# labicon/dp-ilqr

Measured on AMD Instinct MI355X. Metric: ilqr_subproblems_per_sec, higher is better.
Workload: dtype f64; 1 GPU; cfg2: batches of 1024 independent 5-agent DoubleIntDynamics4D iLQR sub-problems per GPU per step, T=50, scripts/analysis.py scenario distribution, tol=1e-3, n_lqr_iter=50; 2468 steps = 2527232 distinct seeds per GPU, window of 6144 in flight; 1 repetition(s) of the job on disjoint seeds, the median is reported; batch_per_gpu=1024, window=6144, n_x=20, n_u=10, horizon=50, parallelism=single GPU

## Files before the change

### dpilqr_amd/_lib.py

```python
import ctypes as C
import os
from pathlib import Path

HERE = Path(__file__).resolve().parent


def route_env(name):
    return os.environ.get(name) if os.environ.get("DPILQR_DEBUG_ROUTES") == "1" else None


def route_flag(name):
    return route_env(name) is not None


LIB_PATH = Path(route_env("DPILQR_LIB")) if route_env("DPILQR_LIB") else HERE / "libdpilqr_hip.so"

i32, i64, f64, vp = C.c_int32, C.c_int64, C.c_double, C.c_void_p

OK, EINVAL, EUNSUPPORTED, EHIP, ENOGPU, EWORKSPACE = 0, -1, -2, -3, -4, -5
N_ALPHA = 10
ABI_VERSION = 4
STATUS_ACTIVE, STATUS_CONVERGED, STATUS_LINESEARCH_FAILED, STATUS_MAX_ITER, STATUS_SINGULAR, STATUS_KILLED, STATUS_FAULT = 0, 1, 2, 3, 4, 5, 6


class BatchDesc(C.Structure):
    _fields_ = [("B", i32), ("k", i32), ("n_s", i32), ("n_c", i32), ("T", i32), ("uniform_model", i32),
                ("dt", f64), ("w_ref", f64), ("w_prox", f64),
                ("model", vp), ("model_bstride", i64), ("n_dims", vp), ("n_dims_bstride", i64),
                ("xf", vp), ("xf_bstride", i64), ("Q", vp), ("Q_bstride", i64), ("R", vp), ("R_bstride", i64),
                ("Qf", vp), ("Qf_bstride", i64), ("radius", vp), ("radius_bstride", i64)]


class DpilqrError(RuntimeError):
    def __init__(self, code, msg):
        super().__init__(f"libdpilqr_hip error {code}: {msg}")
        self.code = code


_DP = C.POINTER(BatchDesc)
SIGNATURES = {
    "dpilqr_abi_version": (i32, []),
    "dpilqr_last_error": (C.c_char_p, []),
    "dpilqr_device_info": (i32, [i32, C.POINTER(i32), C.POINTER(i32), C.c_char_p, i32]),
    "dpilqr_model_dims": (i32, [i32, C.POINTER(i32), C.POINTER(i32)]),
    "dpilqr_model_f": (i32, [i32, i32, vp, vp, vp, vp, vp]),
    "dpilqr_model_integrate": (i32, [i32, i32, vp, vp, vp, f64, vp, vp]),
    "dpilqr_model_linearize": (i32, [i32, i32, vp, vp, vp, f64, vp, vp, vp]),
    "dpilqr_cost_eval": (i32, [_DP, i32, vp, vp, i32, vp, vp]),
    "dpilqr_tile_layout": (i32, [i32, i32, C.POINTER(i64 * 7), C.POINTER(i64 * 7), C.POINTER(i64)]),
    "dpilqr_make_tiles": (i32, [_DP, vp, vp, vp, vp, vp, vp]),
    "dpilqr_rollout": (i32, [_DP, vp, vp, vp, vp, vp]),
    "dpilqr_backward_pass_tiles": (i32, [i32, i32, i32, i32, vp, vp, vp, vp, vp, vp, vp, vp]),
    "dpilqr_backward_pass_tiles_blocks": (i32, [i32, i32, i32, i32, i32, i32, vp, vp, vp, vp, vp, vp, vp, vp]),
    "dpilqr_tiles_bytes": (i64, [i32, i32, i32, i32]),
    "dpilqr_backward_pass": (i32, [_DP, vp, vp, vp, vp, vp, vp, vp]),
    "dpilqr_backward_pass_fused": (i32, [_DP, vp, vp, vp, vp, vp, vp, vp]),
    "dpilqr_forward_pass": (i32, [_DP, vp, vp, vp, vp, vp, i32, vp, vp, vp, vp]),
    "dpilqr_alphas": (i32, [C.POINTER(f64 * N_ALPHA)]),
    "dpilqr_solve_workspace_bytes": (i64, [_DP, i32, i32]),
    "dpilqr_solver_create": (i32, [C.POINTER(vp)]),
    "dpilqr_solver_destroy": (i32, [vp]),
    "dpilqr_solver_set_progress": (i32, [vp, vp, vp]),
    "dpilqr_solve_batch": (i32, [vp, _DP, vp, vp, i32, f64, f64, i32, vp, i64, vp, vp, vp, vp, vp, vp, vp, vp, vp]),
    "dpilqr_solve_enqueue": (i32, [_DP, vp, vp, i32, f64, f64, i32, vp, i64, vp, vp, vp, vp, vp, vp, vp, vp, i32, i32, vp]),
    "dpilqr_solve_iterations_bound": (i64, [_DP, i32, i32]),
    "dpilqr_rollout_f32": (i32, [_DP, vp, vp, vp, vp, vp]),
    "dpilqr_backward_pass_workspace_bytes": (i64, [_DP, i32]),
    "dpilqr_backward_pass_f32": (i32, [_DP, vp, vp, vp, vp, vp, vp, vp]),
    "dpilqr_forward_pass_f32": (i32, [_DP, vp, vp, vp, vp, vp, i32, vp, vp, vp, vp]),
    "dpilqr_solve_workspace_bytes_f32": (i64, [_DP, i32, i32]),
    "dpilqr_solve_batch_f32": (i32, [vp, _DP, vp, vp, i32, f64, f64, i32, vp, i64, vp, vp, vp, vp, vp, vp, vp, vp, vp]),
    "dpilqr_debug_stamps": (i32, [vp]),
    "dpilqr_profile_enable": (i32, [vp, i32]),
    "dpilqr_profile_read": (i32, [vp, C.POINTER(f64 * 4), C.POINTER(i64 * 4), C.POINTER(i64 * 4), i32]),
    "dpilqr_profile_read_sweep": (i32, [vp, i32, C.POINTER(f64), C.POINTER(i64), C.POINTER(i64), i32]),
    "dpilqr_pairwise_graph": (i32, [i32, i32, i32, i32, vp, vp, vp, vp]),
    "dpilqr_dispatch_graph": (i32, [i32, i32, i32, i32, vp, vp, i64, vp, vp, vp, vp, vp, vp, vp, vp, vp]),
    "dpilqr_dispatch_gather": (i32, [i32, i32, i32, i32, i32, i32, vp, i32, i32, vp, vp, vp, vp, i64, vp, vp, vp, vp, vp]),
    "dpilqr_dispatch_gather_params": (i32, [i32, i32, i32, i32, vp, vp, vp, vp]),
    "dpilqr_dispatch_stitch": (i32, [i32, i32, i32, i32, i32, vp, vp, vp, vp, vp, vp, vp, vp]),
    "dpilqr_dispatch_pack_rows": (i32, [i32, i32, i32, i32, i32, vp, vp, vp, vp, vp, vp, vp, vp, i64, vp]),
    "dpilqr_dispatch_scatter_rows": (i32, [i64, i32, i32, i32, i32, vp, i64, vp, vp, vp]),
    "dpilqr_random_setup": (i32, [i32, i64, i32, i32, i32, f64, f64, vp, vp, vp]),
}

_PLAN = [_DP, vp, vp, vp]
_CLOSED_LOOP_ARGS = {"rollout": [i32] + [vp] * 9,
                     "advance": [i32, vp, i32, i32, i32] + [vp] * 12}
EXT_SIGNATURES = {f"dpilqr_policy_{kind}{form}": (i32, _PLAN + ([i32, vp] if "_dec" in form else []) + rest)
                  for kind, rest in _CLOSED_LOOP_ARGS.items() for form in ("", "_large", "_dec", "_dec_team")}
EXT_SIGNATURES["dpilqr_dispatch_stitch_policy"] = (i32, [i32, i32, i32, i32, i32, i32, vp, vp, vp, vp, vp, vp, vp, vp, vp, vp])

SWARM_SIGNATURES = {
    "dpilqr_dispatch_graph_wide": (i32, SIGNATURES["dpilqr_dispatch_graph"][1][:-1] + [i32, vp]),
    "dpilqr_dispatch_gather_wide": (i32, SIGNATURES["dpilqr_dispatch_gather"][1][:-1] + [i32, vp]),
    "dpilqr_dispatch_stitch_wide": (i32, SIGNATURES["dpilqr_dispatch_stitch"][1][:-1] + [i32, vp]),
    "dpilqr_rollout_wide": (i32, [_DP, vp, vp, vp, vp, vp, vp, vp]),
}

SWARM_POLICY_SIGNATURES = {
    "dpilqr_dispatch_stitch_policy_wide": (i32, EXT_SIGNATURES["dpilqr_dispatch_stitch_policy"][1][:-1] + [i32, vp]),
    "dpilqr_policy_rollout_dec_wide": (i32, EXT_SIGNATURES["dpilqr_policy_rollout_dec_team"][1][:-1] + [i32, vp]),
}

SWARM_ADVANCE_SIGNATURES = {
    "dpilqr_policy_advance_dec_wide": (i32, EXT_SIGNATURES["dpilqr_policy_advance_dec_team"][1][:-1] + [i32, vp]),
    "dpilqr_cost_eval_wide": (i32, list(SIGNATURES["dpilqr_cost_eval"][1])),
}

ORDER_SIGNATURES = {
    "dpilqr_cost_keys": (i32, [_DP, vp, vp, vp, vp, vp]),
    "dpilqr_order_list": (i32, [vp, vp, vp, i32, i32, i32, i32, vp, vp]),
    "dpilqr_order_position": (i32, [i32, i32, i32, i32, i32]),
}
ORDER_SPREAD, ORDER_GROUPED = 1, 2

_GW = SWARM_SIGNATURES["dpilqr_dispatch_graph_wide"][1]
NEAREST_SIGNATURES = {"dpilqr_dispatch_graph_nearest": (i32, _GW[:8] + [i32] + _GW[8:15] + [vp] + _GW[15:])}

SWARM_STUDY_SIGNATURES = {
    "dpilqr_trial_inputs": (i32, [i32, C.c_int64, vp, i32, i32, i32, C.c_double, C.c_double, i32, i32, i32, C.c_double, vp, vp, vp, vp, vp]),
}
TRIAL_INPUTS_LDS = 37888

SEPARATED_SIGNATURES = {
    "dpilqr_setup_separate": (i32, [i32, i32, i32, i32, C.c_double, C.c_double, i32, vp, vp, vp, vp]),
}
SETUP_SEPARATE_MAX_ITER = 4096
SETUP_SEPARATE_LDS = 8232

MAX_AGENTS = 64
MAX_TEAM = 256


class BucketResults(C.Structure):
    _fields_ = [("X", vp * (MAX_AGENTS + 1)), ("U", vp * (MAX_AGENTS + 1)), ("first", i32 * (MAX_AGENTS + 1)),
                ("count", i32 * (MAX_AGENTS + 1))]


class BucketGains(C.Structure):
    _fields_ = [("K", vp * (MAX_AGENTS + 1))]


_lib = None


def load():
    global _lib
    if _lib is None:
        if not LIB_PATH.exists():
            raise ImportError(f"{LIB_PATH} is missing: build it with `python -c 'import __graft_entry__ as g; g.build()'` "
                              "(hipcc --offload-arch=gfx950).  dpilqr_amd has no CPU fallback.")
        lib = C.CDLL(str(LIB_PATH))
        for name, (res, args) in {**SIGNATURES, **EXT_SIGNATURES, **SWARM_SIGNATURES, **SWARM_POLICY_SIGNATURES, **SWARM_ADVANCE_SIGNATURES,
                                   **ORDER_SIGNATURES, **NEAREST_SIGNATURES, **SWARM_STUDY_SIGNATURES, **SEPARATED_SIGNATURES}.items():
            fn = getattr(lib, name)
            fn.restype = res
            fn.argtypes = args
        if lib.dpilqr_abi_version() != ABI_VERSION:
            raise ImportError(f"{LIB_PATH}: ABI version {lib.dpilqr_abi_version()}, this binding is for {ABI_VERSION}")
        _lib = lib
    return _lib


def check(rc):
    if rc < 0:
        raise DpilqrError(rc, load().dpilqr_last_error().decode())
    return rc


def alphas():
    a = (f64 * N_ALPHA)()
    check(load().dpilqr_alphas(C.byref(a)))
    return list(a)


TILE_PARTS = ["A", "B", "Lxx", "Lux", "Luu", "Lx", "Lu"]


def tile_layout(n_x, n_u):
    off, ld = (i64 * 7)(), (i64 * 7)()
    stride = i64(0)
    check(load().dpilqr_tile_layout(n_x, n_u, C.byref(off), C.byref(ld), C.byref(stride)))
    return {p: (off[i], ld[i]) for i, p in enumerate(TILE_PARTS)}, stride.value


PROFILE_CLASSES = {"tiles": 1, "riccati": 2, "forward": 4, "rollout": 8}


def profile_enable(on=True, classes=None):
    mask = 0 if not classes else sum(PROFILE_CLASSES[c] for c in classes)
    return load().dpilqr_profile_enable(solver(), int(bool(on)) | (mask << 1))


def profile_read(reset=True):
    ms, ln, it = (f64 * 4)(), (i64 * 4)(), (i64 * 4)()
    check(load().dpilqr_profile_read(solver(), C.byref(ms), C.byref(ln), C.byref(it), int(bool(reset))))
    names = ["tiles", "riccati", "forward", "rollout"]
    return {n: dict(ms=ms[i], launches=ln[i], items=it[i]) for i, n in enumerate(names)}


def profile_read_sweep(waves, reset=True):
    ms, ln, it = f64(), i64(), i64()
    check(load().dpilqr_profile_read_sweep(solver(), int(waves), C.byref(ms), C.byref(ln), C.byref(it), int(bool(reset))))
    return dict(ms=ms.value, launches=ln.value, items=it.value)


import threading

_solvers = threading.local()


def solver():
    import torch
    dev = torch.cuda.current_device()
    table = getattr(_solvers, "table", None)
    if table is None:
        table = _solvers.table = {}
        import atexit
        atexit.register(_destroy_solvers, table)
    if dev not in table:
        h = vp()
        check(load().dpilqr_solver_create(C.byref(h)))
        table[dev] = h
    return table[dev]


PROGRESS_FN = C.CFUNCTYPE(None, vp, i32, i32)


class progress_callback:

    def __init__(self, fn):
        self.error = None

        def call(user, done, total):
            if self.error is not None:
                return
            try:
                fn(int(done), int(total))
            except BaseException as e:
                self.error = e

        self._c = PROGRESS_FN(call) if fn is not None else None

    def __enter__(self):
        if self._c is not None:
            check(load().dpilqr_solver_set_progress(solver(), C.cast(self._c, vp), None))
        return self

    def __exit__(self, *exc):
        if self._c is not None:
            check(load().dpilqr_solver_set_progress(solver(), None, None))
        if self.error is not None and exc[0] is None:
            raise self.error
        return False


def _destroy_solvers(table):
    lib = _lib
    if lib is not None:
        for h in table.values():
            lib.dpilqr_solver_destroy(h)
    table.clear()


_device_ok = None


def require_gpu():
    global _device_ok
    if _device_ok is None:
        import torch
        if not torch.cuda.is_available():
            raise DpilqrError(ENOGPU, "torch.cuda.is_available() is False: dpilqr_amd needs an MI355X (no CPU fallback)")
        check(load().dpilqr_device_info(torch.cuda.current_device(), None, None, None, 0))
        _device_ok = True
    return True
```

### dpilqr_amd/csrc/admit_order.hpp

```cpp
#pragma once
#include <cstdint>

#if defined(__HIPCC__)
#include <hip/hip_runtime.h>
#define DPILQR_HD __host__ __device__
#else
#define DPILQR_HD
#endif

namespace dpilqr {

enum CostOrder : int { kOrderOff = 0, kOrderSpread = 1, kOrderGrouped = 2 };
constexpr int kDefaultCostOrder = kOrderSpread;
enum CostKey : int { kKeyNearCount = 0, kKeyDenseSteps = 1 };
constexpr int kDefaultCostKey = kKeyDenseSteps;

constexpr int kOrderMinLive = 1024;
constexpr int kOrderClasses = 64;

struct SweepDeal {
    int n, n_cus, waves, per_layer, layers, rounds, lo, extra;
    DPILQR_HD SweepDeal(int n_, int n_cus_, int waves_) : n(n_), n_cus(n_cus_), waves(waves_) {
        const int lpr = waves / 4;
        per_layer = 4 * n_cus;
        layers = (n + per_layer - 1) / per_layer;
        rounds = (layers + lpr - 1) / lpr;
        lo = rounds > 0 ? layers / rounds : 0;
        extra = rounds > 0 ? layers - lo * rounds : 0;
    }
    DPILQR_HD int layers_of(int round) const { return lo + (round < extra ? 1 : 0); }
    DPILQR_HD int first_layer(int round) const { return round * lo + (round < extra ? round : extra); }
    DPILQR_HD int round_of_layer(int layer) const {
        const int head = extra * (lo + 1);
        return layer < head ? layer / (lo + 1) : extra + (layer - head) / (lo > 0 ? lo : 1);
    }
    DPILQR_HD int slot(int round, int cu, int wave) const {
        if (round >= rounds || wave >= 4 * layers_of(round)) return -1;
        const int s = (first_layer(round) + (wave >> 2)) * per_layer + (wave & 3) * n_cus + cu;
        return s < n ? s : -1;
    }
};

DPILQR_HD inline int order_position(int rank, const SweepDeal& D, int order) {
    if (order != kOrderGrouped) return rank;
    const int round = D.round_of_layer(rank / D.per_layer);
    const int f = D.first_layer(round), m = D.layers_of(round);
    const int q = rank - f * D.per_layer;
    int base = 4 * m, e = 0;
    if (round == D.rounds - 1) {
        const int rem = D.n - (D.layers - 1) * D.per_layer;
        base = 4 * (m - 1) + rem / D.n_cus;
        e = rem % D.n_cus;
    }
    int cu, w;
    if (q < e * (base + 1)) { cu = q / (base + 1); w = q - cu * (base + 1); }
    else { const int q2 = q - e * (base + 1), per = base > 0 ? base : 1; cu = e + q2 / per; w = q2 - (cu - e) * per; }
    return (f + (w >> 2)) * D.per_layer + (w & 3) * D.n_cus + cu;
}

DPILQR_HD inline int order_class(int key, int T) {
    const int top = T + 1;
    const int c = top < kOrderClasses ? key : (int)((int64_t)key * (kOrderClasses - 1) / top);
    return c < 0 ? 0 : (c > kOrderClasses - 1 ? kOrderClasses - 1 : c);
}

#if defined(__HIPCC__) && defined(DPILQR_ADMIT_ORDER_KERNELS)

constexpr int kKeyStagedAgents = 5;
__global__ void __launch_bounds__(256) k_cost_keys(const double* __restrict__ X, const double* __restrict__ radius, int64_t radius_bstride,
                                                   const int32_t* __restrict__ list, const int32_t* __restrict__ count, int B, int T, int k,
                                                   int min_live, int32_t* __restrict__ key, int32_t* __restrict__ key_dense) {
    __shared__ double2 sP[4][64 * kKeyStagedAgents];
    const int n = count ? *count : B;
    if (n <= min_live) return;
    const int wave = (int)threadIdx.x >> 6, lane = threadIdx.x & 63;
    const int pos = (int)blockIdx.x * 4 + wave;
    if (pos >= n) return;
    const int b = list ? list[pos] : pos;
    if (b < 0 || b >= B) return;
    const double r = radius[(int64_t)b * radius_bstride];
    const double lim = r * r * (1.0 + 1e-12);
    const int nx = 4 * k;
    const double* Xb = X + (int64_t)b * (T + 1) * nx;
    const bool staged = k <= kKeyStagedAgents;
    int cnt = 0, dense = 0;
    for (int t0 = 0; t0 <= T; t0 += 64) {
        const int rows = min(64, T + 1 - t0);
        bool near = false;
        if (staged) {
            const double2* src = reinterpret_cast<const double2*>(Xb + (int64_t)t0 * nx);
            for (int e = lane; e < rows * k; e += 64) sP[wave][e] = src[2 * e];
            __builtin_amdgcn_wave_barrier();
            asm volatile("" ::: "memory");
            if (lane < rows) {
                double2 p[kKeyStagedAgents];
#pragma unroll
                for (int i = 0; i < kKeyStagedAgents; ++i) p[i] = sP[wave][lane * k + min(i, k - 1)];
#pragma unroll
                for (int i = 0; i < kKeyStagedAgents; ++i)
#pragma unroll
                    for (int j = i + 1; j < kKeyStagedAgents; ++j) {
                        const double ddx = p[i].x - p[j].x, ddy = p[i].y - p[j].y;
                        const double s2 = ddx * ddx + ddy * ddy;
                        near = near || (j < k && !(s2 > lim));
                    }
            }
            __builtin_amdgcn_wave_barrier();
            asm volatile("" ::: "memory");
        } else if (lane < rows) {
            const double* row = Xb + (int64_t)(t0 + lane) * nx;
            for (int i = 0; i < k; ++i)
                for (int j = i + 1; j < k; ++j) {
                    const double ddx = row[4 * i] - row[4 * j], ddy = row[4 * i + 1] - row[4 * j + 1];
                    const double s2 = ddx * ddx + ddy * ddy;
                    near = near || !(s2 > lim);
                }
        }
        const unsigned long long mask = __builtin_amdgcn_ballot_w64(near);
        cnt += __popcll(mask);
        if (mask) dense = t0 + 64 - __clzll(mask);
    }
    if (lane == 0) {
        if (key) key[pos] = cnt;
        if (key_dense) key_dense[pos] = dense;
    }
}

__global__ void __launch_bounds__(1024) k_order_list(const int32_t* __restrict__ src, int32_t* __restrict__ dst, const int32_t* __restrict__ count,
                                                     const int32_t* __restrict__ key, int T, int n_cus, int waves, int order, int min_live) {
    static_assert(kOrderClasses == 64, "the prefix sums below are one wavefront's, a bin per lane");
    __shared__ int hist[kOrderClasses], cursor[kOrderClasses];
    const int n = *count;
    if (n <= min_live || order == kOrderOff) {
        for (int i = threadIdx.x; i < n; i += blockDim.x) dst[i] = src[i];
        return;
    }
    if (threadIdx.x < kOrderClasses) hist[threadIdx.x] = 0;
    __syncthreads();
    for (int i = threadIdx.x; i < n; i += blockDim.x) atomicAdd(&hist[kOrderClasses - 1 - order_class(key[i], T)], 1);
    __syncthreads();
    if (threadIdx.x < kOrderClasses) {
        const int own = hist[threadIdx.x];
        int run = own;
        for (int off = 1; off < kOrderClasses; off <<= 1) {
            const int below = __shfl_up(run, off);
            if ((int)threadIdx.x >= off) run += below;
        }
        cursor[threadIdx.x] = run - own;
    }
    __syncthreads();
    const SweepDeal deal(n, n_cus, waves);
    for (int i = threadIdx.x; i < n; i += blockDim.x) {
        const int rank = atomicAdd(&cursor[kOrderClasses - 1 - order_class(key[i], T)], 1);
        const int pos = order_position(rank, deal, order);
        if (pos >= 0 && pos < n) dst[pos] = src[i];
    }
}

#endif

}
```

### dpilqr_amd/csrc/dpilqr_hip.hip

```cpp
#include <hip/hip_runtime.h>

#include <cstdarg>
#include <cstdio>
#include <algorithm>
#include <cstdlib>
#include <cstring>
#include <new>
#include <vector>

#include "dpilqr_hip.h"
#include "admit_order.hpp"
#include "launch.hpp"
#include "models.hpp"
#include "tiles.hpp"

namespace dpilqr {

static thread_local char g_err[512] = "";

int32_t fail(int32_t code, const char* fmt, ...) {
    va_list ap;
    va_start(ap, fmt);
    vsnprintf(g_err, sizeof(g_err), fmt, ap);
    va_end(ap);
    return code;
}
const char* last_error() { return g_err; }

const char* route_env(const char* name) {
    static const bool open = [] { const char* g = std::getenv("DPILQR_DEBUG_ROUTES"); return g && g[0] == '1' && g[1] == 0; }();
    return open ? std::getenv(name) : nullptr;
}

int device_cus() {
    static int cus_of[64] = {0};
    int dev = 0;
    if (hipGetDevice(&dev) != hipSuccess || dev < 0 || dev >= 64) return 256;
    if (cus_of[dev] == 0) {
        int n = 0;
        if (hipDeviceGetAttribute(&n, hipDeviceAttributeMultiprocessorCount, dev) != hipSuccess || n <= 0) n = 256;
        cus_of[dev] = n;
    }
    return cus_of[dev];
}

}

using namespace dpilqr;

namespace {

constexpr int kMaxAgents = 64;

int family_nc(int ns) { return ns == 3 ? 2 : ns == 4 ? 2 : ns == 5 ? 2 : ns == 6 ? 3 : ns == 12 ? 4 : -1; }

int32_t check_family5(const dpilqr_batch_desc* d, bool f32) {
    if (d->n_s != 5) return DPILQR_OK;
    if (f32) return fail(DPILQR_EUNSUPPORTED, "the fp32 arm does not serve the five-state family (BikeDynamics5D)");
    if (d->k * d->n_s > 60)
        return fail(DPILQR_EUNSUPPORTED, "k=%d BikeDynamics5D agents (n_x=%d): the five-state family is served up to 12 agents (n_x <= 60)",
                    d->k, d->k * d->n_s);
    return DPILQR_OK;
}

int32_t check_desc(const dpilqr_batch_desc* d, int max_k = kMaxAgents) {
    if (!d) return fail(DPILQR_EINVAL, "desc is NULL");
    if (d->B < 0 || d->k < 1 || d->T < 1) return fail(DPILQR_EINVAL, "bad sizes B=%d k=%d T=%d", d->B, d->k, d->T);
    if (d->k > max_k) return fail(DPILQR_EUNSUPPORTED, "k=%d agents per sub-problem exceeds %d", d->k, max_k);
    if (family_nc(d->n_s) != d->n_c)
        return fail(DPILQR_EINVAL, "(n_s,n_c)=(%d,%d) is not a model family; expected (3,2),(4,2),(5,2),(6,3),(12,4)", d->n_s, d->n_c);
    if (d->B > 0 && (!d->model || !d->n_dims || !d->xf || !d->Q || !d->R || !d->Qf || !d->radius))
        return fail(DPILQR_EINVAL, "desc holds a NULL device pointer");
    const uintptr_t ints = reinterpret_cast<uintptr_t>(d->model) | reinterpret_cast<uintptr_t>(d->n_dims);
    const uintptr_t dbls = reinterpret_cast<uintptr_t>(d->xf) | reinterpret_cast<uintptr_t>(d->Q) | reinterpret_cast<uintptr_t>(d->R) |
                           reinterpret_cast<uintptr_t>(d->Qf) | reinterpret_cast<uintptr_t>(d->radius);
    if (d->B > 0 && (ints % alignof(int32_t) != 0 || dbls % alignof(double) != 0))
        return fail(DPILQR_EINVAL, "desc holds a device pointer that is not aligned to its element type");
    return check_family5(d, false);
}

hipStream_t as_stream(void* s) { return reinterpret_cast<hipStream_t>(s); }

void alpha_table(double* a) {
    static const uint32_t bits[DPILQR_N_ALPHA] = {0x3f800000u, 0x3f68ba2eu, 0x3f2ed9f7u, 0x3ed92350u, 0x3e5eda27u,
                                                  0x3dbd05a8u, 0x3d04808du, 0x3c19864au, 0x3b13029cu, 0x39e8ae70u};
    for (int i = 0; i < DPILQR_N_ALPHA; ++i) {
        float f;
        memcpy(&f, &bits[i], 4);
        a[i] = (double)f;
    }
}

__global__ void k_init_state(int B, double* mu, double* delta, int32_t* status, int32_t* n_bwd, int32_t* n_fwd,
                             int32_t* singular, int32_t* counts, int n_counts, double* alphas_dev, double a0, double a1,
                             double a2, double a3, double a4, double a5, double a6, double a7, double a8, double a9) {
    const int i = blockIdx.x * blockDim.x + threadIdx.x;
    if (i < B) {
        mu[i] = 1.0; delta[i] = 2.0; status[i] = DPILQR_STATUS_ACTIVE; n_bwd[i] = 0; n_fwd[i] = 0; singular[i] = 0;
    }
    if (i < n_counts) counts[i] = 0;
    if (i == 0) {
        alphas_dev[0] = a0; alphas_dev[1] = a1; alphas_dev[2] = a2; alphas_dev[3] = a3; alphas_dev[4] = a4;
        alphas_dev[5] = a5; alphas_dev[6] = a6; alphas_dev[7] = a7; alphas_dev[8] = a8; alphas_dev[9] = a9;
    }
}

__global__ void k_admit(int32_t* list, int32_t* count, int32_t* next_count, int32_t* admitted, int B, int window,
                        int32_t* mail, int want_prefix, int64_t* t_admit, const int32_t* fault) {
    const int base = *count, first = *admitted;
    const int n_new = min(B - first, window - base);
    __shared__ int lowest;
    if (threadIdx.x == 0) lowest = first;
    __syncthreads();
    for (int i = threadIdx.x; i < n_new; i += blockDim.x) list[base + i] = first + i;
    if (t_admit && n_new > 0) {
        const int64_t now = (int64_t)__builtin_amdgcn_s_memrealtime();
        for (int i = threadIdx.x; i < n_new; i += blockDim.x) t_admit[first + i] = now;
    }
    if (mail && want_prefix) {
        int lo = first;
        for (int i = threadIdx.x; i < base; i += blockDim.x) lo = min(lo, list[i]);
        for (int off = 32; off > 0; off >>= 1) lo = min(lo, __shfl_down(lo, off));
        if ((threadIdx.x & 63) == 0) atomicMin(&lowest, lo);
        __syncthreads();
    }
    if (threadIdx.x == 0) {
        *count = base + n_new; *admitted = first + n_new; *next_count = 0;
        if (mail) { mail[0] = base + n_new; mail[1] = first + n_new; mail[2] = want_prefix ? lowest : 0; mail[3] = *fault; }
    }
}

__global__ void k_copy_f64(int n, const double* src, double* dst) {
    const int i = blockIdx.x * blockDim.x + threadIdx.x;
    if (i < n) dst[i] = src[i];
}

__global__ void k_finish_status(int B, int32_t* status) {
    const int i = blockIdx.x * blockDim.x + threadIdx.x;
    if (i < B && status[i] == DPILQR_STATUS_ACTIVE) status[i] = DPILQR_STATUS_MAX_ITER;
}

constexpr int kCountRing = 4;

struct SolveShape {
    bool big;
    size_t elem;
    bool fused;
};

struct SolveWorkspace {
    size_t tiles, K, d, Xc, Uc, mu, delta, J_star, J_last, alphas, singular, lists, counts, t_admit, total;
    SolveWorkspace(const dpilqr_batch_desc& D, int W, bool gains_in_ws, SolveShape sh) {
        const size_t B = D.B, n = (size_t)D.k * D.n_s, m = (size_t)D.k * D.n_c, T = D.T, Wn = W, e = sh.elem;
        const TileLayout L((int)n, (int)m);
        auto al = [](size_t x) { return (x + 255) & ~(size_t)255; };
        size_t o = 0;
        tiles = o;    o = al(o + (sh.big ? e * Wn * (size_t)riccati_big_scratch_elems((int)n, (int)m)
                                         : (sh.fused ? 0 : sizeof(double) * Wn * (T + 1) * L.stride)));
        K = o;        o = al(o + (gains_in_ws ? e * Wn * T * m * n : 0));
        d = o;        o = al(o + (gains_in_ws ? e * Wn * T * m : 0));
        Xc = o;       o = al(o + e * Wn * DPILQR_N_ALPHA * (T + 1) * n);
        Uc = o;       o = al(o + e * Wn * DPILQR_N_ALPHA * T * m);
        mu = o;       o = al(o + sizeof(double) * B);
        delta = o;    o = al(o + sizeof(double) * B);
        J_star = o;   o = al(o + sizeof(double) * B);
        J_last = o;   o = al(o + sizeof(double) * B);
        alphas = o;   o = al(o + sizeof(double) * DPILQR_N_ALPHA);
        singular = o; o = al(o + sizeof(int32_t) * B);
        lists = o;    o = al(o + sizeof(int32_t) * 2 * Wn);
        counts = o;   o = al(o + sizeof(int32_t) * (kCountRing + 2));
        t_admit = o;  o = al(o + sizeof(int64_t) * B);
        total = o;
    }
};
constexpr int kMaxLqrIter = 4096;
constexpr int kMaxGlobalIter = 1 << 20;

int window_of(const dpilqr_batch_desc& D, int window) { return (window <= 0 || window > D.B) ? (D.B > 0 ? D.B : 1) : window; }

constexpr int kHostLag = 3, kMailRing = kHostLag + 1, kMailWords = 4;

struct Profiler {
    bool on = false;
    int mask = 0xF;
    bool skip = false;
    double ms[4] = {0, 0, 0, 0};
    int64_t launches[4] = {0, 0, 0, 0}, items[4] = {0, 0, 0, 0};
    double sweep_ms[3] = {0, 0, 0};
    int64_t sweep_launches[3] = {0, 0, 0}, sweep_items[3] = {0, 0, 0};
    std::vector<hipEvent_t> pool;
    struct Rec { int cls, iter; size_t e0; int tag; };
    std::vector<Rec> recs;
    size_t used = 0;
    ~Profiler() {
        for (auto& e : pool) (void)hipEventDestroy(e);
    }
    hipEvent_t next() {
        if (used == pool.size()) {
            hipEvent_t e;
            if (hipEventCreate(&e) != hipSuccess) return nullptr;
            pool.push_back(e);
        }
        return pool[used++];
    }
    void begin(int cls, int iter, hipStream_t st) {
        skip = !on || !((mask >> cls) & 1);
        if (skip) return;
        recs.push_back({cls, iter, used, 0});
        hipEvent_t e = next();
        if (e) (void)hipEventRecord(e, st);
    }
    void end(hipStream_t st, int tag = 0) {
        if (skip) return;
        hipEvent_t e = next();
        if (e) (void)hipEventRecord(e, st);
        recs.back().tag = tag;
    }
    void drop() { recs.clear(); used = 0; }
    void collect(const std::vector<int32_t>& active, int B) {
        if (!on) { drop(); return; }
        for (const Rec& r : recs) {
            float t = 0.f;
            if (r.e0 + 1 < pool.size() && hipEventElapsedTime(&t, pool[r.e0], pool[r.e0 + 1]) == hipSuccess) {
                const int64_t n_it = (r.iter < 0) ? B : (r.iter < (int)active.size() ? active[r.iter] : 0);
                ms[r.cls] += t;
                launches[r.cls] += 1;
                items[r.cls] += n_it;
                if (r.cls == 1 && (r.tag == 4 || r.tag == 8 || r.tag == 12)) {
                    const int v = r.tag / 4 - 1;
                    sweep_ms[v] += t; sweep_launches[v] += 1; sweep_items[v] += n_it;
                }
            }
        }
        drop();
    }
};

}

struct dpilqr_solver {
    int device = -1;
    int32_t* host = nullptr;
    int32_t* dev = nullptr;
    std::vector<int32_t> hist;
    hipEvent_t ev[kMailRing] = {};
    Profiler prof;
    dpilqr_progress_fn progress = nullptr;
    void* progress_user = nullptr;
    int32_t init() {
        HIP_TRY(hipGetDevice(&device));
        HIP_TRY(hipHostMalloc(reinterpret_cast<void**>(&host), sizeof(int32_t) * kMailWords * kMailRing, hipHostMallocDefault));
        HIP_TRY(hipHostGetDevicePointer(reinterpret_cast<void**>(&dev), host, 0));
        for (auto& e : ev) HIP_TRY(hipEventCreateWithFlags(&e, hipEventDisableTiming));
        return DPILQR_OK;
    }
    void release() {
        if (host) (void)hipHostFree(host);
        host = nullptr;
        for (auto& e : ev) {
            if (e) (void)hipEventDestroy(e);
            e = nullptr;
        }
    }
    ~dpilqr_solver() { release(); }
};

namespace {

thread_local dpilqr_solver g_default_solver;

int32_t default_solver(dpilqr_solver** out) {
    int dev = 0;
    HIP_TRY(hipGetDevice(&dev));
    if (g_default_solver.host && g_default_solver.device != dev) g_default_solver.release();
    if (!g_default_solver.host) {
        int32_t rc = g_default_solver.init();
        if (rc) return rc;
    }
    *out = &g_default_solver;
    return DPILQR_OK;
}

__global__ void k_normalise_lists(int32_t* lists, int32_t* counts, int window, int it_end, int src) {
    const int cs = it_end % kCountRing;
    __shared__ int n_sh;
    if (threadIdx.x == 0) n_sh = counts[cs];
    __syncthreads();
    const int n = n_sh;
    if (src == 1)
        for (int i = threadIdx.x; i < n; i += blockDim.x) lists[i] = lists[window + i];
    __syncthreads();
    if (threadIdx.x == 0) {
        for (int c = 0; c < kCountRing; ++c) counts[c] = 0;
        counts[0] = n;
    }
}

template <typename R> struct Passes;
template <> struct Passes<double> {
    static int32_t forward(const dpilqr_batch_desc& D, int mode, const double* x0, double* X, double* U, const double* K,
                           const double* d, const double* alphas, int ngrp, double* Xc, double* Uc, double* Jc,
                           const SolveState& S, const int32_t* items, const int32_t* n_items, int grid, hipStream_t st) {
        return launch_forward(D, mode, x0, X, U, K, d, alphas, ngrp, Xc, Uc, Jc, S, items, n_items, grid, st);
    }
    static int32_t sweep_big(const dpilqr_batch_desc& D, const double* X, const double* U, const double* mu, double* K, double* d,
                             int32_t* sing, const int32_t* items, const int32_t* n_items, int grid, int by_item, void* scratch,
                             hipStream_t st) {
        return launch_riccati_big_f64(D, X, U, mu, K, d, sing, items, n_items, grid, by_item, scratch, st);
    }
};
template <> struct Passes<float> {
    static int32_t forward(const dpilqr_batch_desc& D, int mode, const float* x0, float* X, float* U, const float* K,
                           const float* d, const double* alphas, int ngrp, float* Xc, float* Uc, double* Jc,
                           const SolveState& S, const int32_t* items, const int32_t* n_items, int grid, hipStream_t st) {
        return launch_forward_big_f32(D, mode, x0, X, U, K, d, alphas, ngrp, Xc, Uc, Jc, S, items, n_items, grid, st);
    }
    static int32_t sweep_big(const dpilqr_batch_desc& D, const float* X, const float* U, const double* mu, float* K, float* d,
                             int32_t* sing, const int32_t* items, const int32_t* n_items, int grid, int by_item, void* scratch,
                             hipStream_t st) {
        return launch_riccati_big_f32(D, X, U, mu, K, d, sing, items, n_items, grid, by_item, scratch, st);
    }
};

template <typename R>
SolveShape shape_of(const dpilqr_batch_desc& D) {
    const bool big = sizeof(R) == 4 || uses_big_path(D.k * D.n_s);
    return SolveShape{big, sizeof(R), !big && fused_sweep_applies(D) && !solve_prefers_records(D)};
}

template <typename R>
int32_t solve_impl(dpilqr_solver* solver, const dpilqr_batch_desc* desc, const R* x0, R* U, int32_t n_lqr_iter, double tol,
                   double t_kill, int32_t window, void* workspace, int64_t workspace_bytes, R* X, double* J, int32_t* status,
                   int32_t* n_bwd, int32_t* n_fwd, double* trace, R* K_out, R* d_out, int32_t n_global_iter,
                   int32_t resume, hipStream_t st) {
    int32_t rc = check_desc(desc);
    if (!rc) rc = check_family5(desc, sizeof(R) == 4);
    if (rc) return rc;
    if (desc->B == 0) return DPILQR_OK;
    if (!x0 || !U || !X || !J || !status || !n_bwd || !n_fwd || !workspace)
        return fail(DPILQR_EINVAL, "solve_batch: NULL pointer");
    if ((K_out == nullptr) != (d_out == nullptr)) return fail(DPILQR_EINVAL, "solve_batch: K_out and d_out go together");
    if (n_lqr_iter < 0 || n_lqr_iter > kMaxLqrIter) return fail(DPILQR_EINVAL, "solve_batch: n_lqr_iter=%d", n_lqr_iter);
    if (!solver && n_global_iter < 0) return fail(DPILQR_EINVAL, "solve_enqueue: n_global_iter=%d", n_global_iter);
    const dpilqr_batch_desc& D = *desc;
    const int Wn = window_of(D, window);
    const bool gains_by_item = K_out != nullptr;
    const SolveShape sh = shape_of<R>(D);
    const SolveWorkspace W(D, Wn, !gains_by_item, sh);
    if (workspace_bytes < (int64_t)W.total)
        return fail(DPILQR_EWORKSPACE, "solve_batch: workspace %lld B < required %zu B", (long long)workspace_bytes, W.total);
    if (solver) {
        int dev = 0;
        HIP_TRY(hipGetDevice(&dev));
        if (dev != solver->device)
            return fail(DPILQR_EINVAL, "solve_batch: the solver belongs to device %d, the current device is %d", solver->device, dev);
    }
    char* ws = static_cast<char*>(workspace);
    double* tiles = reinterpret_cast<double*>(ws + W.tiles);
    R* K = gains_by_item ? K_out : reinterpret_cast<R*>(ws + W.K);
    R* d = gains_by_item ? d_out : reinterpret_cast<R*>(ws + W.d);
    double* alphas = reinterpret_cast<double*>(ws + W.alphas);
    R* Xc = reinterpret_cast<R*>(ws + W.Xc);
    R* Uc = reinterpret_cast<R*>(ws + W.Uc);
    int32_t* lists = reinterpret_cast<int32_t*>(ws + W.lists);
    int32_t* counts = reinterpret_cast<int32_t*>(ws + W.counts);
    int32_t* singular = reinterpret_cast<int32_t*>(ws + W.singular);
    SolveState S{};
    S.mu = reinterpret_cast<double*>(ws + W.mu);
    S.delta = reinterpret_cast<double*>(ws + W.delta);
    S.J_star = reinterpret_cast<double*>(ws + W.J_star);
    S.J_last = reinterpret_cast<double*>(ws + W.J_last);
    S.status = status; S.n_bwd = n_bwd; S.n_fwd = n_fwd; S.trace = trace; S.singular = singular;
    S.n_lqr_iter = n_lqr_iter; S.tol = tol; S.gains_by_item = gains_by_item ? 1 : 0;
    int64_t* t_admit = nullptr;
    S.t_admit = nullptr; S.t_kill_ticks = 0;
    if (t_kill > 0.0) {
        int dev_now = 0, khz = 0;
        HIP_TRY(hipGetDevice(&dev_now));
        if (hipDeviceGetAttribute(&khz, hipDeviceAttributeWallClockRate, dev_now) != hipSuccess || khz <= 0) khz = 100000;
        const double ticks = t_kill * 1e3 * (double)khz;
        S.t_kill_ticks = ticks < 1.0 ? 1 : (ticks > 9e18 ? (int64_t)9e18 : (int64_t)ticks);
        t_admit = reinterpret_cast<int64_t*>(ws + W.t_admit);
        S.t_admit = t_admit;
    }
    const int n = D.k * D.n_s, m = D.k * D.n_c;
    Profiler none;
    Profiler& prof = solver ? solver->prof : none;
    if (solver) solver->hist.clear();
    auto bail = [&](int32_t code) {
        (void)hipStreamSynchronize(st);
        prof.drop();
        return code;
    };

    int32_t* admitted_dev = counts + kCountRing;
    S.fault = counts + kCountRing + 1;
    static const bool no_static = route_flag("DPILQR_TILES_NO_STATIC");
    const int um = hint_model(D);
    const bool fused = sh.fused;
    const bool static_part = !fused && !sh.big && !no_static && D.R_bstride == 0 &&
                             (um == kDoubleInt4D || um == kDoubleInt6D || um == kHumanLin6D);
    if (!resume) {
        double a[DPILQR_N_ALPHA];
        alpha_table(a);
        const int init_n = D.B > kCountRing + 2 ? D.B : kCountRing + 2;
        hipLaunchKernelGGL(k_init_state, dim3((init_n + 255) / 256), dim3(256), 0, st, D.B, S.mu, S.delta, status, n_bwd, n_fwd,
                           singular, counts, kCountRing + 2, alphas, a[0], a[1], a[2], a[3], a[4], a[5], a[6], a[7], a[8], a[9]);
        HIP_TRY(hipGetLastError());
        prof.begin(3, -1, st);
        rc = Passes<R>::forward(D, kModeRollout, x0, X, U, nullptr, nullptr, nullptr, 1, nullptr, nullptr, S.J_star, S, nullptr,
                                nullptr, D.B, st);
        if (rc) return bail(rc);
        prof.end(st);
        hipLaunchKernelGGL(k_copy_f64, dim3((D.B + 255) / 256), dim3(256), 0, st, D.B, S.J_star, S.J_last);
        if (n_lqr_iter > 0) {
            if (!fused && hipMemsetAsync(tiles, 0, W.K - W.tiles, st) != hipSuccess) return bail(fail(DPILQR_EHIP, "hipMemsetAsync failed"));
            if (static_part) {
                if constexpr (sizeof(R) == 8) {
                    if ((rc = launch_make_tiles(D, X, U, tiles, nullptr, nullptr, Wn, true, false, st))) return bail(rc);
                }
            }
        }
    }

    static const int order_route = route_flag("DPILQR_NO_COST_ORDER") ? (int)kOrderOff : route_int("DPILQR_COST_ORDER", kDefaultCostOrder);
    static const bool dense_key = !route_flag("DPILQR_NO_DECOUPLED") && route_int("DPILQR_COST_KEY", kDefaultCostKey) == (int)kKeyDenseSteps;
    const int order = (sizeof(R) == 8 && fused && (order_route == kOrderSpread || order_route == kOrderGrouped)) ? order_route : (int)kOrderOff;
    int32_t* keys = reinterpret_cast<int32_t*>(ws + W.Xc);
    int surv = 0;
    size_t n_iterations = 0;
    auto enqueue_iteration = [&](int it, int upper) -> int32_t {
        int32_t* cur = lists + (size_t)surv * Wn;
        int32_t* other = lists + (size_t)(surv ^ 1) * Wn;
        int32_t* cur_n = counts + (it % kCountRing);
        int32_t* nxt_n = counts + ((it + 1) % kCountRing);
        int32_t* mail = solver ? solver->dev + kMailWords * (it % kMailRing) : nullptr;
        hipLaunchKernelGGL(k_admit, dim3(1), dim3(256), 0, st, cur, cur_n, nxt_n, admitted_dev, D.B, Wn, mail,
                           (solver && solver->progress) ? 1 : 0, t_admit, S.fault);
        if (solver) HIP_TRY(hipEventRecord(solver->ev[it % kMailRing], st));
        int32_t r = DPILQR_OK;
        const int order_waves = order ? fused_sweep_tier(D, upper) : 0;
        if (order_waves > 0) {
            if constexpr (sizeof(R) == 8) {
                if ((r = launch_cost_keys(D, X, cur, cur_n, upper, kOrderMinLive, dense_key ? nullptr : keys, dense_key ? keys : nullptr, st))) return r;
                if ((r = launch_order_list(cur, other, cur_n, keys, D.T, device_cus(), order_waves, order, kOrderMinLive, st))) return r;
            }
            S.next_items = cur;
            cur = other;
        } else {
            S.next_items = other;
            surv ^= 1;
        }
        S.next_count = nxt_n;
        if (fused) {
            if constexpr (sizeof(R) == 8) {
                prof.begin(1, it, st);
                if ((r = launch_riccati_fused(D, X, U, S.mu, K, d, singular, cur, cur_n, upper, S.gains_by_item, st))) return r;
                prof.end(st, g_sweep_waves);
            }
        } else if (!sh.big) {
            if constexpr (sizeof(R) == 8) {
                prof.begin(0, it, st);
                if ((r = launch_make_tiles(D, X, U, tiles, cur, cur_n, upper, true, static_part, st))) return r;
                prof.end(st);
                prof.begin(1, it, st);
                if ((r = launch_riccati(D.B, D.T, n, m, tiles, S.mu, K, d, singular, cur, cur_n, upper, S.gains_by_item, D.n_s,
                                        D.n_c, st)))
                    return r;
                prof.end(st, g_sweep_waves);
            }
        } else {
            prof.begin(1, it, st);
            if ((r = Passes<R>::sweep_big(D, X, U, S.mu, K, d, singular, cur, cur_n, upper, S.gains_by_item, tiles, st))) return r;
            prof.end(st, 0);
        }
        prof.begin(2, it, st);
        if ((r = Passes<R>::forward(D, kModeLineSearch, nullptr, X, U, K, d, alphas, DPILQR_N_ALPHA, Xc, Uc, nullptr, S, cur, cur_n,
                                    upper, st)))
            return r;
        prof.end(st);
        return DPILQR_OK;
    };

    if (n_lqr_iter > 0 && solver) {
        int upper = Wn;
        int32_t reported = 0;
        for (int it = 0; it < kMaxGlobalIter; ++it) {
            n_iterations = (size_t)it + 1;
            if ((rc = enqueue_iteration(it, upper))) return bail(rc);
            bool done = false;
            if (it >= kHostLag) {
                const int slot = (it - kHostLag) % kMailRing;
                if (hipEventSynchronize(solver->ev[slot]) != hipSuccess) return bail(fail(DPILQR_EHIP, "hipEventSynchronize failed"));
                const int32_t act = solver->host[kMailWords * slot], adm = solver->host[kMailWords * slot + 1];
                const int32_t prefix = solver->host[kMailWords * slot + 2];
                solver->hist.push_back(act);
                if (solver->progress && prefix > reported) { reported = prefix; solver->progress(solver->progress_user, prefix, D.B); }
                done = (adm >= D.B && act == 0);
                upper = (adm >= D.B) ? std::min(Wn, std::max(act, 1)) : Wn;
            }
            if (done) break;
            if (it + 1 == kMaxGlobalIter) return bail(fail(DPILQR_EUNSUPPORTED, "solve_batch: more than %d global iterations", kMaxGlobalIter));
        }
    } else if (n_lqr_iter > 0) {
        for (int it = 0; it < n_global_iter; ++it)
            if ((rc = enqueue_iteration(it, Wn))) return rc;
        if (n_global_iter > 0)
            hipLaunchKernelGGL(k_normalise_lists, dim3(1), dim3(256), 0, st, lists, counts, Wn, n_global_iter, surv);
    }
    hipLaunchKernelGGL(k_copy_f64, dim3((D.B + 255) / 256), dim3(256), 0, st, D.B, S.J_last, J);
    if (n_lqr_iter == 0) hipLaunchKernelGGL(k_finish_status, dim3((D.B + 255) / 256), dim3(256), 0, st, D.B, status);
    HIP_TRY(hipGetLastError());
    if (!solver) return DPILQR_OK;
    if (hipStreamSynchronize(st) != hipSuccess) return bail(fail(DPILQR_EHIP, "hipStreamSynchronize failed"));
    if (n_lqr_iter > 0) {
        for (size_t j = solver->hist.size(); j < n_iterations; ++j) solver->hist.push_back(solver->host[kMailWords * (j % kMailRing)]);
    }
    prof.collect(solver->hist, D.B);
    if (solver->progress) solver->progress(solver->progress_user, D.B, D.B);
    if (n_lqr_iter > 0) {
        int32_t faulted = 0;
        for (int j = 0; j < kMailRing; ++j) faulted = std::max(faulted, solver->host[kMailWords * j + 3]);
        if (faulted > 0)
            return fail(DPILQR_EHIP, "solve_batch: the device gave up %d of %d items (status DPILQR_STATUS_FAULT: a hand-over inside a "
                                     "team of workgroups expired); every other item's result is valid", faulted, D.B);
    }
    return DPILQR_OK;
}

}

extern "C" {

int32_t dpilqr_abi_version(void) { return DPILQR_ABI_VERSION; }
const char* dpilqr_last_error(void) { return last_error(); }

int32_t dpilqr_device_info(int32_t dev, int32_t* n_cu, int32_t* lds_bytes, char* arch, int32_t arch_len) {
    int count = 0;
    if (hipGetDeviceCount(&count) != hipSuccess || count <= 0) return fail(DPILQR_ENOGPU, "no HIP device visible");
    if (dev < 0 || dev >= count) return fail(DPILQR_EINVAL, "device %d out of range (%d visible)", dev, count);
    hipDeviceProp_t p;
    HIP_TRY(hipGetDeviceProperties(&p, dev));
    if (n_cu) *n_cu = p.multiProcessorCount;
    if (lds_bytes) *lds_bytes = (int32_t)p.maxSharedMemoryPerMultiProcessor;
    if (arch && arch_len > 0) { strncpy(arch, p.gcnArchName, arch_len - 1); arch[arch_len - 1] = 0; }
    if (strncmp(p.gcnArchName, "gfx950", 6) != 0)
        return fail(DPILQR_ENOGPU, "device %d is %s; this library is built for gfx950 only", dev, p.gcnArchName);
    return DPILQR_OK;
}

int32_t dpilqr_model_dims(int32_t model, int32_t* n_s, int32_t* n_c) {
    if (model < 0 || model >= kNumModels || model_ns(model) < 0 || !n_s || !n_c) return fail(DPILQR_EINVAL, "unknown model %d", model);
    *n_s = model_ns(model);
    *n_c = model_nc(model);
    return DPILQR_OK;
}

static int32_t model_op(int op, int32_t n, int32_t ns, const int32_t* model, const double* x, const double* u, double dt,
                        double* o1, double* o2, void* stream) {
    if (n < 0 || !model || !x || !u || !o1 || (op == 2 && !o2)) return fail(DPILQR_EINVAL, "model op: bad argument");
    if (n == 0) return DPILQR_OK;
    return launch_model_op(op, n, ns, model, x, u, dt, o1, o2, as_stream(stream));
}

int32_t dpilqr_model_f(int32_t n, int32_t family_ns, const int32_t* model, const double* x, const double* u,
                       double* x_dot, void* stream) {
    return model_op(0, n, family_ns, model, x, u, 0.0, x_dot, nullptr, stream);
}
int32_t dpilqr_model_integrate(int32_t n, int32_t family_ns, const int32_t* model, const double* x, const double* u,
                               double dt, double* x_new, void* stream) {
    return model_op(1, n, family_ns, model, x, u, dt, x_new, nullptr, stream);
}
int32_t dpilqr_model_linearize(int32_t n, int32_t family_ns, const int32_t* model, const double* x, const double* u,
                               double dt, double* A, double* B, void* stream) {
    return model_op(2, n, family_ns, model, x, u, dt, A, B, stream);
}

int32_t dpilqr_cost_eval(const dpilqr_batch_desc* desc, int32_t n_pts, const double* x, const double* u,
                         int32_t terminal, double* cost, void* stream) {
    int32_t rc = check_desc(desc);
    if (rc) return rc;
    if (n_pts < 0 || !x || !u || !cost) return fail(DPILQR_EINVAL, "cost_eval: bad argument");
    if ((int64_t)desc->B * n_pts == 0) return DPILQR_OK;
    return launch_cost_eval(*desc, n_pts, x, u, terminal, cost, as_stream(stream));
}

int32_t dpilqr_tile_layout(int32_t n_x, int32_t n_u, int64_t offsets[7], int64_t row_strides[7], int64_t* stride) {
    if (n_x < 1 || n_u < 1 || !offsets || !row_strides || !stride) return fail(DPILQR_EINVAL, "tile_layout: bad argument");
    return tile_layout_host(n_x, n_u, offsets, row_strides, stride);
}

int64_t dpilqr_tiles_bytes(int32_t B, int32_t T, int32_t n_x, int32_t n_u) {
    if (B < 0 || T < 1 || n_x < 1 || n_u < 1) return fail(DPILQR_EINVAL, "tiles_bytes: bad argument");
    return (int64_t)sizeof(double) * B * (T + 1) * TileLayout(n_x, n_u).stride;
}

int32_t dpilqr_make_tiles(const dpilqr_batch_desc* desc, const double* X, const double* U, double* tiles,
                          const int32_t* items, const int32_t* n_items, void* stream) {
    int32_t rc = check_desc(desc);
    if (rc) return rc;
    if (!X || !U || !tiles) return fail(DPILQR_EINVAL, "make_tiles: NULL pointer");
    return launch_make_tiles(*desc, X, U, tiles, items, n_items, desc->B, false, false, as_stream(stream));
}

int32_t dpilqr_rollout(const dpilqr_batch_desc* desc, const double* x0, const double* U, double* X, double* J,
                       void* stream) {
    int32_t rc = check_desc(desc);
    if (rc) return rc;
    if (desc->B == 0) return DPILQR_OK;
    if (!x0 || !U || !X || !J) return fail(DPILQR_EINVAL, "rollout: NULL pointer");
    SolveState S{};
    return launch_forward(*desc, kModeRollout, x0, X, const_cast<double*>(U), nullptr, nullptr, nullptr, 1, nullptr,
                          nullptr, J, S, nullptr, nullptr, desc->B, as_stream(stream));
}

int32_t dpilqr_rollout_wide(const dpilqr_batch_desc* desc, const double* x0, const double* U, double* X, double* J,
                            double* min_sep, double* goal_dist, void* stream) {
    const int32_t rc = check_desc(desc, 256);
    if (rc) return rc;
    if (!x0 || !U || !J) return fail(DPILQR_EINVAL, "rollout_wide: NULL pointer");
    uintptr_t dbls = 0;
    for (const double* p : {x0, U, (const double*)X, (const double*)J, (const double*)min_sep, (const double*)goal_dist}) dbls |= reinterpret_cast<uintptr_t>(p);
    if (dbls % alignof(double) != 0) return fail(DPILQR_EINVAL, "rollout_wide: a device pointer is not aligned to its element type");
    return launch_rollout_wide(*desc, x0, U, X, J, min_sep, goal_dist, as_stream(stream));
}

int32_t dpilqr_backward_pass_tiles(int32_t B, int32_t T, int32_t n_x, int32_t n_u, const double* tiles,
                                   const double* mu, double* K, double* d, int32_t* singular, const int32_t* items,
                                   const int32_t* n_items, void* stream) {
    if (B < 0 || T < 1 || n_x < 1 || n_u < 1) return fail(DPILQR_EINVAL, "backward_pass_tiles: bad sizes");
    if (!tiles || !mu || !K || !d) return fail(DPILQR_EINVAL, "backward_pass_tiles: NULL pointer");
    return launch_riccati(B, T, n_x, n_u, tiles, mu, K, d, singular, items, n_items, B, 0, 0, 0, as_stream(stream));
}

int32_t dpilqr_backward_pass_tiles_blocks(int32_t B, int32_t T, int32_t n_x, int32_t n_u, int32_t block_ns,
                                          int32_t block_nc, const double* tiles, const double* mu, double* K,
                                          double* d, int32_t* singular, const int32_t* items,
                                          const int32_t* n_items, void* stream) {
    if (B < 0 || T < 1 || n_x < 1 || n_u < 1) return fail(DPILQR_EINVAL, "backward_pass_tiles_blocks: bad sizes");
    if (!tiles || !mu || !K || !d) return fail(DPILQR_EINVAL, "backward_pass_tiles_blocks: NULL pointer");
    if (block_ns < 0 || block_nc < 0 || (block_ns > 0 && (block_nc < 1 || n_x % block_ns || n_u % block_nc ||
                                                          n_x / block_ns != n_u / block_nc)))
        return fail(DPILQR_EINVAL, "backward_pass_tiles_blocks: n_x=%d, n_u=%d are not k blocks of %d, %d", n_x, n_u,
                    block_ns, block_nc);
    return launch_riccati(B, T, n_x, n_u, tiles, mu, K, d, singular, items, n_items, B, 0, block_ns, block_nc,
                          as_stream(stream));
}

int64_t dpilqr_backward_pass_workspace_bytes(const dpilqr_batch_desc* desc, int32_t elem_bytes) {
    if (!desc || desc->B < 0 || desc->k < 1 || desc->T < 1 || (elem_bytes != 4 && elem_bytes != 8))
        return fail(DPILQR_EINVAL, "backward_pass_workspace_bytes: bad argument");
    const int n = desc->k * desc->n_s, m = desc->k * desc->n_c;
    if (elem_bytes == 4 || uses_big_path(n)) return (int64_t)elem_bytes * desc->B * riccati_big_scratch_elems(n, m);
    return (int64_t)sizeof(double) * desc->B * (desc->T + 1) * TileLayout(n, m).stride;
}

int32_t dpilqr_backward_pass(const dpilqr_batch_desc* desc, const double* X, const double* U, const double* mu,
                             double* K, double* d, double* tiles_workspace, void* stream) {
    int32_t rc = check_desc(desc);
    if (rc) return rc;
    if (desc->B == 0) return DPILQR_OK;
    if (!X || !U || !mu || !K || !d || !tiles_workspace) return fail(DPILQR_EINVAL, "backward_pass: NULL pointer");
    const int n = desc->k * desc->n_s, m = desc->k * desc->n_c;
    if (uses_big_path(n)) {
        HIP_TRY(hipMemsetAsync(tiles_workspace, 0, sizeof(double) * desc->B * (size_t)riccati_big_scratch_elems(n, m), as_stream(stream)));
        return launch_riccati_big_f64(*desc, X, U, mu, K, d, nullptr, nullptr, nullptr, desc->B, 0, tiles_workspace, as_stream(stream));
    }
    rc = launch_make_tiles(*desc, X, U, tiles_workspace, nullptr, nullptr, desc->B, false, false, as_stream(stream));
    if (rc) return rc;
    return launch_riccati(desc->B, desc->T, n, m, tiles_workspace, mu, K, d, nullptr, nullptr, nullptr, desc->B, 0, desc->n_s,
                          desc->n_c, as_stream(stream));
}

int32_t dpilqr_backward_pass_fused(const dpilqr_batch_desc* desc, const double* X, const double* U, const double* mu, double* K,
                                   double* d, int32_t* singular, void* stream) {
    int32_t rc = check_desc(desc);
    if (rc) return rc;
    if (desc->B == 0) return DPILQR_OK;
    if (!X || !U || !mu || !K || !d) return fail(DPILQR_EINVAL, "backward_pass_fused: NULL pointer");
    if (!fused_sweep_applies(*desc))
        return fail(DPILQR_EUNSUPPORTED, "backward_pass_fused: needs 6..15 four-state, 1..10 six-state, 1..6 CarDynamics3D or 1..4 BikeDynamics5D agents, or at most five "
                                         "DoubleIntDynamics4D / UnicycleDynamics4D agents with n_dims = 2 (uniform_model hints)");
    rc = launch_riccati_fused(*desc, X, U, mu, K, d, singular, nullptr, nullptr, desc->B, 0, as_stream(stream));
    return rc == DPILQR_EUNSUPPORTED ? fail(rc, "backward_pass_fused: no instantiation for n_x=%d", desc->k * desc->n_s) : rc;
}

int32_t dpilqr_backward_pass_f32(const dpilqr_batch_desc* desc, const float* X, const float* U, const double* mu, float* K,
                                 float* d, void* workspace, void* stream) {
    int32_t rc = check_desc(desc);
    if (!rc) rc = check_family5(desc, true);
    if (rc) return rc;
    if (desc->B == 0) return DPILQR_OK;
    if (!X || !U || !mu || !K || !d || !workspace) return fail(DPILQR_EINVAL, "backward_pass_f32: NULL pointer");
    const int n = desc->k * desc->n_s, m = desc->k * desc->n_c;
    HIP_TRY(hipMemsetAsync(workspace, 0, sizeof(float) * desc->B * (size_t)riccati_big_scratch_elems(n, m), as_stream(stream)));
    return launch_riccati_big_f32(*desc, X, U, mu, K, d, nullptr, nullptr, nullptr, desc->B, 0, workspace, as_stream(stream));
}

int32_t dpilqr_rollout_f32(const dpilqr_batch_desc* desc, const float* x0, const float* U, float* X, double* J, void* stream) {
    int32_t rc = check_desc(desc);
    if (!rc) rc = check_family5(desc, true);
    if (rc) return rc;
    if (desc->B == 0) return DPILQR_OK;
    if (!x0 || !U || !X || !J) return fail(DPILQR_EINVAL, "rollout_f32: NULL pointer");
    SolveState S{};
    return launch_forward_big_f32(*desc, kModeRollout, x0, X, const_cast<float*>(U), nullptr, nullptr, nullptr, 1, nullptr, nullptr,
                                  J, S, nullptr, nullptr, desc->B, as_stream(stream));
}

int32_t dpilqr_forward_pass_f32(const dpilqr_batch_desc* desc, const float* X, const float* U, const float* K, const float* d,
                                const double* alphas, int32_t n_alpha, float* Xn, float* Un, double* Jn, void* stream) {
    int32_t rc = check_desc(desc);
    if (!rc) rc = check_family5(desc, true);
    if (rc) return rc;
    if (desc->B == 0) return DPILQR_OK;
    if (!X || !U || !K || !d || !alphas || !Xn || !Un || !Jn) return fail(DPILQR_EINVAL, "forward_pass_f32: NULL pointer");
    if (n_alpha < 1) return fail(DPILQR_EINVAL, "forward_pass_f32: n_alpha=%d", n_alpha);
    SolveState S{};
    return launch_forward_big_f32(*desc, kModeCandidates, nullptr, const_cast<float*>(X), const_cast<float*>(U), K, d, alphas,
                                  n_alpha, Xn, Un, Jn, S, nullptr, nullptr, desc->B, as_stream(stream));
}

int32_t dpilqr_forward_pass(const dpilqr_batch_desc* desc, const double* X, const double* U, const double* K,
                            const double* d, const double* alphas, int32_t n_alpha, double* Xn, double* Un, double* Jn,
                            void* stream) {
    int32_t rc = check_desc(desc);
    if (rc) return rc;
    if (!X || !U || !K || !d || !alphas || !Xn || !Un || !Jn) return fail(DPILQR_EINVAL, "forward_pass: NULL pointer");
    if (n_alpha < 1) return fail(DPILQR_EINVAL, "forward_pass: n_alpha=%d", n_alpha);
    SolveState S{};
    return launch_forward(*desc, kModeCandidates, nullptr, const_cast<double*>(X), const_cast<double*>(U), K, d, alphas,
                          n_alpha, Xn, Un, Jn, S, nullptr, nullptr, desc->B, as_stream(stream));
}

static int32_t check_policy_args(const char* who, const dpilqr_batch_desc* desc, const PolicyRolloutArgs& a, int max_k = kMaxAgents) {
    const int32_t rc = check_desc(desc, max_k);
    if (rc) return rc;
    const PolicyPlan& p = a.plan;
    if (!p.X || !p.U || !p.K || !a.x0s || !a.J) return fail(DPILQR_EINVAL, "%s: NULL pointer", who);
    if (a.n_samples <= 0) return fail(DPILQR_EINVAL, "%s: n_samples=%d", who, a.n_samples);
    const double* const doubles[] = {p.X, p.U, p.K, a.x0s, a.J, a.W, a.u_lim, a.Xs, a.Us, a.min_sep, a.goal_dist};
    uintptr_t dbls = 0;
    for (const double* q : doubles) dbls |= reinterpret_cast<uintptr_t>(q);
    return dbls % alignof(double) == 0 ? DPILQR_OK : fail(DPILQR_EINVAL, "%s: a device pointer is not aligned to its element type", who);
}

static int32_t check_advance_args(const char* who, const dpilqr_batch_desc* desc, const PolicyAdvanceArgs& a, int max_k = kMaxAgents) {
    const int32_t rc = check_desc(desc, max_k);
    if (rc) return rc;
    const PolicyPlan& p = a.plan;
    if (!p.X || !p.U || !a.x_cur || !a.n_done || !a.X_exec || !a.U_exec || !a.J_exec || !a.min_sep || !a.dist_left || !a.U_next || !a.X_next)
        return fail(DPILQR_EINVAL, "%s: NULL pointer", who);
    if (a.h < 1 || a.h > desc->T) return fail(DPILQR_EINVAL, "%s: h=%d, a round executes 1 .. T = %d steps", who, a.h, desc->T);
    if (a.L < 1) return fail(DPILQR_EINVAL, "%s: L=%d", who, a.L);
    if (a.n_d < 1 || a.n_d > desc->n_s) return fail(DPILQR_EINVAL, "%s: n_d=%d, an agent has n_s = %d states", who, a.n_d, desc->n_s);
    if (a.n_scen < desc->B) return fail(DPILQR_EINVAL, "%s: n_scen=%d for B = %d items", who, a.n_scen, desc->B);
    const double* const doubles[] = {p.X, p.U, p.K, a.W, a.u_lim, a.x_cur, a.X_exec, a.U_exec, a.J_exec, a.min_sep, a.dist_left, a.U_next, a.X_next};
    uintptr_t dbls = 0;
    for (const double* q : doubles) dbls |= reinterpret_cast<uintptr_t>(q);
    const uintptr_t ints = reinterpret_cast<uintptr_t>(a.scen) | reinterpret_cast<uintptr_t>(a.n_done);
    return dbls % alignof(double) == 0 && ints % alignof(int32_t) == 0
               ? DPILQR_OK : fail(DPILQR_EINVAL, "%s: a device pointer is not aligned to its element type", who);
}

static int32_t check_masks(const char* who, const PolicyPlan& p) {
    if ((p.K && !p.nbr_bits) || reinterpret_cast<uintptr_t>(p.nbr_bits) % alignof(uint64_t) != 0)
        return fail(DPILQR_EINVAL, "%s: nbr_bits is a NULL pointer or not aligned to its element type", who);
    return DPILQR_OK;
}

int32_t dpilqr_policy_rollout(const dpilqr_batch_desc* desc, const double* X, const double* U, const double* K, int32_t n_samples,
                              const double* x0s, const double* W, const double* u_lim, double* Xs, double* Us, double* J,
                              double* min_sep, double* goal_dist, void* stream) {
    const PolicyRolloutArgs a{{X, U, K, 0, nullptr}, n_samples, x0s, W, u_lim, Xs, Us, J, min_sep, goal_dist};
    const int32_t rc = check_policy_args("policy_rollout", desc, a);
    return rc ? rc : launch_policy_rollout(*desc, a, as_stream(stream));
}

int32_t dpilqr_policy_rollout_large(const dpilqr_batch_desc* desc, const double* X, const double* U, const double* K, int32_t n_samples,
                                    const double* x0s, const double* W, const double* u_lim, double* Xs, double* Us, double* J,
                                    double* min_sep, double* goal_dist, void* stream) {
    const PolicyRolloutArgs a{{X, U, K, 0, nullptr}, n_samples, x0s, W, u_lim, Xs, Us, J, min_sep, goal_dist};
    const int32_t rc = check_policy_args("policy_rollout_large", desc, a);
    return rc ? rc : launch_policy_rollout_large(*desc, a, as_stream(stream));
}

int32_t dpilqr_policy_rollout_dec(const dpilqr_batch_desc* desc, const double* X, const double* U_ff, const double* Kc, int32_t kc_max,
                                  const uint64_t* nbr_bits, int32_t n_samples, const double* x0s, const double* W, const double* u_lim,
                                  double* Xs, double* Us, double* J, double* min_sep, double* goal_dist, void* stream) {
    const PolicyRolloutArgs a{{X, U_ff, Kc, kc_max, nbr_bits}, n_samples, x0s, W, u_lim, Xs, Us, J, min_sep, goal_dist};
    int32_t rc = check_policy_args("policy_rollout_dec", desc, a);
    if (!rc) rc = check_masks("policy_rollout_dec", a.plan);
    return rc ? rc : launch_policy_rollout_dec(*desc, a, as_stream(stream));
}

int32_t dpilqr_policy_rollout_dec_team(const dpilqr_batch_desc* desc, const double* X, const double* U_ff, const double* Kc, int32_t kc_max,
                                       const uint64_t* nbr_bits, int32_t n_samples, const double* x0s, const double* W, const double* u_lim,
                                       double* Xs, double* Us, double* J, double* min_sep, double* goal_dist, void* stream) {
    const PolicyRolloutArgs a{{X, U_ff, Kc, kc_max, nbr_bits}, n_samples, x0s, W, u_lim, Xs, Us, J, min_sep, goal_dist};
    int32_t rc = check_policy_args("policy_rollout_dec_team", desc, a);
    if (!rc) rc = check_masks("policy_rollout_dec_team", a.plan);
    return rc ? rc : launch_policy_rollout_dec_team(*desc, a, as_stream(stream));
}

int32_t dpilqr_policy_rollout_dec_wide(const dpilqr_batch_desc* desc, const double* X, const double* U_ff, const double* Kc, int32_t kc_max,
                                       const uint64_t* nbr_bits, int32_t n_samples, const double* x0s, const double* W, const double* u_lim,
                                       double* Xs, double* Us, double* J, double* min_sep, double* goal_dist, int32_t n_words, void* stream) {
    const PolicyRolloutArgs a{{X, U_ff, Kc, kc_max, nbr_bits}, n_samples, x0s, W, u_lim, Xs, Us, J, min_sep, goal_dist};
    int32_t rc = check_policy_args("policy_rollout_dec_wide", desc, a, DPILQR_MAX_TEAM);
    if (!rc) rc = check_masks("policy_rollout_dec_wide", a.plan);
    return rc ? rc : launch_policy_rollout_dec_wide(*desc, a, n_words, as_stream(stream));
}

int32_t dpilqr_policy_advance(const dpilqr_batch_desc* desc, const double* X, const double* U, const double* K, int32_t h,
                              const int32_t* scen, int32_t n_scen, int32_t L, int32_t n_d, const double* W, const double* u_lim,
                              double* x_cur, int32_t* n_done, double* X_exec, double* U_exec, double* J_exec, double* min_sep,
                              double* dist_left, double* U_next, double* X_next, void* stream) {
    const PolicyAdvanceArgs a{{X, U, K, 0, nullptr}, h, scen, n_scen, L, n_d, W, u_lim, x_cur, n_done, X_exec, U_exec, J_exec, min_sep,
                              dist_left, U_next, X_next};
    const int32_t rc = check_advance_args("policy_advance", desc, a);
    return rc ? rc : launch_policy_advance(*desc, a, as_stream(stream));
}

int32_t dpilqr_policy_advance_large(const dpilqr_batch_desc* desc, const double* X, const double* U, const double* K, int32_t h,
                                    const int32_t* scen, int32_t n_scen, int32_t L, int32_t n_d, const double* W, const double* u_lim,
                                    double* x_cur, int32_t* n_done, double* X_exec, double* U_exec, double* J_exec, double* min_sep,
                                    double* dist_left, double* U_next, double* X_next, void* stream) {
    const PolicyAdvanceArgs a{{X, U, K, 0, nullptr}, h, scen, n_scen, L, n_d, W, u_lim, x_cur, n_done, X_exec, U_exec, J_exec, min_sep,
                              dist_left, U_next, X_next};
    int32_t rc = check_advance_args("policy_advance_large", desc, a);
    if (rc == DPILQR_EUNSUPPORTED && desc->n_s == 5)
        rc = fail(DPILQR_EUNSUPPORTED, "policy_advance_large: the (5, 2) family is served up to n_x = 60, by dpilqr_policy_advance; "
                                       "served here are the (4, 2), (6, 3) and (12, 4) families with 60 < n_x <= 240, k <= 20");
    return rc ? rc : launch_policy_advance_large(*desc, a, as_stream(stream));
}

int32_t dpilqr_policy_advance_dec(const dpilqr_batch_desc* desc, const double* X, const double* U_ff, const double* Kc,
                                  int32_t kc_max, const uint64_t* nbr_bits, int32_t h, const int32_t* scen, int32_t n_scen,
                                  int32_t L, int32_t n_d, const double* W, const double* u_lim, double* x_cur, int32_t* n_done,
                                  double* X_exec, double* U_exec, double* J_exec, double* min_sep, double* dist_left,
                                  double* U_next, double* X_next, void* stream) {
    const PolicyAdvanceArgs a{{X, U_ff, Kc, kc_max, nbr_bits}, h, scen, n_scen, L, n_d, W, u_lim, x_cur, n_done, X_exec, U_exec, J_exec,
                              min_sep, dist_left, U_next, X_next};
    int32_t rc = check_advance_args("policy_advance_dec", desc, a);
    if (!rc) rc = check_masks("policy_advance_dec", a.plan);
    if (!rc) rc = check_kc_max("policy_advance_dec", *desc, kc_max);
    return rc ? rc : launch_policy_advance(*desc, a, as_stream(stream));
}

int32_t dpilqr_policy_advance_dec_team(const dpilqr_batch_desc* desc, const double* X, const double* U_ff, const double* Kc,
                                       int32_t kc_max, const uint64_t* nbr_bits, int32_t h, const int32_t* scen, int32_t n_scen,
                                       int32_t L, int32_t n_d, const double* W, const double* u_lim, double* x_cur, int32_t* n_done,
                                       double* X_exec, double* U_exec, double* J_exec, double* min_sep, double* dist_left,
                                       double* U_next, double* X_next, void* stream) {
    const PolicyAdvanceArgs a{{X, U_ff, Kc, kc_max, nbr_bits}, h, scen, n_scen, L, n_d, W, u_lim, x_cur, n_done, X_exec, U_exec, J_exec,
                              min_sep, dist_left, U_next, X_next};
    int32_t rc = check_advance_args("policy_advance_dec_team", desc, a);
    if (!rc) rc = check_masks("policy_advance_dec_team", a.plan);
    return rc ? rc : launch_policy_advance_dec_team(*desc, a, as_stream(stream));
}

int32_t dpilqr_policy_advance_dec_wide(const dpilqr_batch_desc* desc, const double* X, const double* U_ff, const double* Kc,
                                       int32_t kc_max, const uint64_t* nbr_bits, int32_t h, const int32_t* scen, int32_t n_scen,
                                       int32_t L, int32_t n_d, const double* W, const double* u_lim, double* x_cur, int32_t* n_done,
                                       double* X_exec, double* U_exec, double* J_exec, double* min_sep, double* dist_left,
                                       double* U_next, double* X_next, int32_t n_words, void* stream) {
    const PolicyAdvanceArgs a{{X, U_ff, Kc, kc_max, nbr_bits}, h, scen, n_scen, L, n_d, W, u_lim, x_cur, n_done, X_exec, U_exec, J_exec,
                              min_sep, dist_left, U_next, X_next};
    int32_t rc = check_advance_args("policy_advance_dec_wide", desc, a, DPILQR_MAX_TEAM);
    if (!rc) rc = check_masks("policy_advance_dec_wide", a.plan);
    return rc ? rc : launch_policy_advance_dec_wide(*desc, a, n_words, as_stream(stream));
}

int32_t dpilqr_cost_eval_wide(const dpilqr_batch_desc* desc, int32_t n_pts, const double* x, const double* u,
                              int32_t terminal, double* cost, void* stream) {
    int32_t rc = check_desc(desc, DPILQR_MAX_TEAM);
    if (rc) return rc;
    if (n_pts < 0 || !x || !u || !cost) return fail(DPILQR_EINVAL, "cost_eval_wide: bad argument");
    if ((int64_t)desc->B * n_pts == 0) return DPILQR_OK;
    return launch_cost_eval(*desc, n_pts, x, u, terminal, cost, as_stream(stream));
}

int32_t dpilqr_alphas(double* alphas_host) {
    if (!alphas_host) return fail(DPILQR_EINVAL, "alphas: NULL pointer");
    alpha_table(alphas_host);
    return DPILQR_OK;
}

int64_t dpilqr_solve_workspace_bytes(const dpilqr_batch_desc* desc, int32_t window, int32_t gains_in_workspace) {
    if (!desc || desc->B < 0 || desc->k < 1 || desc->T < 1) return fail(DPILQR_EINVAL, "solve_workspace_bytes: bad desc");
    return (int64_t)SolveWorkspace(*desc, window_of(*desc, window), gains_in_workspace != 0, shape_of<double>(*desc)).total;
}
int64_t dpilqr_solve_workspace_bytes_f32(const dpilqr_batch_desc* desc, int32_t window, int32_t gains_in_workspace) {
    if (!desc || desc->B < 0 || desc->k < 1 || desc->T < 1) return fail(DPILQR_EINVAL, "solve_workspace_bytes_f32: bad desc");
    return (int64_t)SolveWorkspace(*desc, window_of(*desc, window), gains_in_workspace != 0, shape_of<float>(*desc)).total;
}

int32_t dpilqr_solver_create(dpilqr_solver** out) {
    if (!out) return fail(DPILQR_EINVAL, "solver_create: NULL pointer");
    dpilqr_solver* s = new (std::nothrow) dpilqr_solver();
    if (!s) return fail(DPILQR_EHIP, "solver_create: out of host memory");
    const int32_t rc = s->init();
    if (rc) { delete s; return rc; }
    *out = s;
    return DPILQR_OK;
}
int32_t dpilqr_solver_destroy(dpilqr_solver* solver) {
    delete solver;
    return DPILQR_OK;
}
int32_t dpilqr_solver_set_progress(dpilqr_solver* solver, dpilqr_progress_fn fn, void* user) {
    if (!solver) {
        const int32_t rc = default_solver(&solver);
        if (rc) return rc;
    }
    solver->progress = fn;
    solver->progress_user = user;
    return DPILQR_OK;
}

int32_t dpilqr_solve_batch(dpilqr_solver* solver, const dpilqr_batch_desc* desc, const double* x0, double* U,
                           int32_t n_lqr_iter, double tol, double t_kill, int32_t window, void* workspace, int64_t workspace_bytes,
                           double* X, double* J, int32_t* status, int32_t* n_bwd, int32_t* n_fwd, double* trace,
                           double* K_out, double* d_out, void* stream) {
    if (!solver) {
        const int32_t rc = default_solver(&solver);
        if (rc) return rc;
    }
    return solve_impl<double>(solver, desc, x0, U, n_lqr_iter, tol, t_kill, window, workspace, workspace_bytes, X, J, status, n_bwd,
                              n_fwd, trace, K_out, d_out, 0, 0, as_stream(stream));
}
int32_t dpilqr_solve_batch_f32(dpilqr_solver* solver, const dpilqr_batch_desc* desc, const float* x0, float* U,
                               int32_t n_lqr_iter, double tol, double t_kill, int32_t window, void* workspace, int64_t workspace_bytes,
                               float* X, double* J, int32_t* status, int32_t* n_bwd, int32_t* n_fwd, double* trace,
                               float* K_out, float* d_out, void* stream) {
    if (!solver) {
        const int32_t rc = default_solver(&solver);
        if (rc) return rc;
    }
    return solve_impl<float>(solver, desc, x0, U, n_lqr_iter, tol, t_kill, window, workspace, workspace_bytes, X, J, status, n_bwd,
                             n_fwd, trace, K_out, d_out, 0, 0, as_stream(stream));
}
int32_t dpilqr_solve_enqueue(const dpilqr_batch_desc* desc, const double* x0, double* U, int32_t n_lqr_iter, double tol,
                             double t_kill, int32_t window, void* workspace, int64_t workspace_bytes, double* X, double* J, int32_t* status,
                             int32_t* n_bwd, int32_t* n_fwd, double* trace, double* K_out, double* d_out,
                             int32_t n_global_iter, int32_t resume, void* stream) {
    return solve_impl<double>(nullptr, desc, x0, U, n_lqr_iter, tol, t_kill, window, workspace, workspace_bytes, X, J, status, n_bwd,
                              n_fwd, trace, K_out, d_out, n_global_iter, resume, as_stream(stream));
}
int64_t dpilqr_solve_iterations_bound(const dpilqr_batch_desc* desc, int32_t window, int32_t n_lqr_iter) {
    if (!desc || desc->B < 0 || n_lqr_iter < 0) return fail(DPILQR_EINVAL, "solve_iterations_bound: bad argument");
    const int64_t W = window_of(*desc, window);
    return ((int64_t)desc->B + W - 1) / W * n_lqr_iter + 1;
}

int32_t dpilqr_debug_stamps(void* buf) {
    int32_t rc = set_stamp_buffer_riccati(buf);
    return rc ? rc : set_stamp_buffer_forward(buf);
}

int32_t dpilqr_cost_keys(const dpilqr_batch_desc* desc, const double* X, const int32_t* items, const int32_t* n_items, int32_t* keys,
                         void* stream) {
    int32_t rc = check_desc(desc);
    if (rc) return rc;
    if (desc->n_s != 4) return fail(DPILQR_EUNSUPPORTED, "cost_keys: n_s=%d, the keys are defined for the four-state family", desc->n_s);
    if (desc->B == 0) return DPILQR_OK;
    if (!X || !keys || ((items == nullptr) != (n_items == nullptr))) return fail(DPILQR_EINVAL, "cost_keys: NULL pointer");
    static const bool second = route_flag("DPILQR_KEYS_DENSE_STEPS");
    return launch_cost_keys(*desc, X, items, n_items, desc->B, -1, second ? nullptr : keys, second ? keys : nullptr, as_stream(stream));
}

int32_t dpilqr_order_list(const int32_t* items, const int32_t* n_items, const int32_t* keys, int32_t T, int32_t n_cus, int32_t waves,
                          int32_t order, int32_t* out, void* stream) {
    if (!items || !n_items || !keys || !out) return fail(DPILQR_EINVAL, "order_list: NULL pointer");
    if (T < 1 || n_cus < 1 || (waves != 4 && waves != 8 && waves != 12) || (order != kOrderSpread && order != kOrderGrouped))
        return fail(DPILQR_EINVAL, "order_list: T=%d n_cus=%d waves=%d order=%d", T, n_cus, waves, order);
    return launch_order_list(items, out, n_items, keys, T, n_cus, waves, order, -1, as_stream(stream));
}

int32_t dpilqr_order_position(int32_t rank, int32_t n, int32_t n_cus, int32_t waves, int32_t order) {
    if (n < 1 || rank < 0 || rank >= n || n_cus < 1 || (waves != 4 && waves != 8 && waves != 12) ||
        (order != kOrderSpread && order != kOrderGrouped))
        return fail(DPILQR_EINVAL, "order_position: rank=%d n=%d n_cus=%d waves=%d order=%d", rank, n, n_cus, waves, order);
    return order_position(rank, SweepDeal(n, n_cus, waves), order);
}

int32_t dpilqr_profile_enable(dpilqr_solver* solver, int32_t enable) {
    Profiler& g_prof = solver ? solver->prof : g_default_solver.prof;
    const int32_t prev = g_prof.on ? 1 : 0;
    g_prof.on = (enable & 1) != 0;
    g_prof.mask = (enable >> 1) & 0xF ? (enable >> 1) & 0xF : 0xF;
    return prev;
}

int32_t dpilqr_profile_read(dpilqr_solver* solver, double ms[4], int64_t launches[4], int64_t items[4], int32_t reset) {
    if (!ms || !launches || !items) return fail(DPILQR_EINVAL, "profile_read: NULL pointer");
    Profiler& g_prof = solver ? solver->prof : g_default_solver.prof;
    for (int c = 0; c < 4; ++c) {
        ms[c] = g_prof.ms[c]; launches[c] = g_prof.launches[c]; items[c] = g_prof.items[c];
        if (reset) { g_prof.ms[c] = 0; g_prof.launches[c] = 0; g_prof.items[c] = 0; }
    }
    return DPILQR_OK;
}

int32_t dpilqr_profile_read_sweep(dpilqr_solver* solver, int32_t waves, double* ms, int64_t* launches, int64_t* items, int32_t reset) {
    if (!ms || !launches || !items) return fail(DPILQR_EINVAL, "profile_read_sweep: NULL pointer");
    if (waves != 4 && waves != 8 && waves != 12) return fail(DPILQR_EINVAL, "profile_read_sweep: waves=%d (4, 8 or 12)", waves);
    const int v = waves / 4 - 1;
    Profiler& g_prof = solver ? solver->prof : g_default_solver.prof;
    *ms = g_prof.sweep_ms[v]; *launches = g_prof.sweep_launches[v]; *items = g_prof.sweep_items[v];
    if (reset) { g_prof.sweep_ms[v] = 0; g_prof.sweep_launches[v] = 0; g_prof.sweep_items[v] = 0; }
    return DPILQR_OK;
}

int32_t dpilqr_pairwise_graph(int32_t S, int32_t N, int32_t k, int32_t n_s, const double* X, const double* radius,
                              int32_t* adj, void* stream) {
    if (S < 0 || N < 1 || k < 1 || n_s < 2 || !X || !radius || !adj) return fail(DPILQR_EINVAL, "pairwise_graph: bad argument");
    if (S == 0) return DPILQR_OK;
    return launch_pairwise_graph(S, N, k, n_s, X, radius, adj, as_stream(stream));
}

}
```

### dpilqr_amd/csrc/forward_wave.hpp

```cpp
#pragma once
#include <hip/hip_runtime.h>

#include "forward.hpp"
#include "wave_util.hpp"

namespace dpilqr {

template <int KA>
struct PairTable {
    int i[KA * (KA - 1) / 2 + 1], j[KA * (KA - 1) / 2 + 1];
    constexpr PairTable() : i{}, j{} {
        int p = 0;
        for (int a = 0; a < KA; ++a)
            for (int b = a + 1; b < KA; ++b) { i[p] = a; j[p] = b; ++p; }
    }
};

__device__ inline int linesearch_decide(const SolveState& S, int b, int ngrp, const double* sJ) {
    const int iter = S.n_bwd[b];
    const double J_star = S.J_star[b];
    int acc = -1;
    for (int i = 0; i < ngrp; ++i)
        if (sJ[i] < J_star) { acc = i; break; }
    const int n_eval = (acc >= 0) ? acc + 1 : ngrp;
    const double J_last = sJ[n_eval - 1];
    const double mu_before = S.mu[b];
    int status = DPILQR_STATUS_ACTIVE;
    double J_new = J_star;
    if (acc >= 0) {
        const bool conv = fabs((J_star - J_last) / J_star) < S.tol;
        J_new = J_last;
        double delta = fmin(1.0, S.delta[b]) / 2.0;
        double mu = mu_before * delta;
        if (mu <= 1e-6) mu = 0.0;
        S.delta[b] = delta; S.mu[b] = mu; S.J_star[b] = J_new;
        if (conv) status = DPILQR_STATUS_CONVERGED;
        else if (solve_time_is_up(S, b)) status = DPILQR_STATUS_KILLED;
        else if (iter + 1 >= S.n_lqr_iter) status = DPILQR_STATUS_MAX_ITER;
    } else {
        status = DPILQR_STATUS_LINESEARCH_FAILED;
    }
    S.J_last[b] = J_last;
    S.n_fwd[b] += n_eval;
    S.n_bwd[b] = iter + 1;
    S.status[b] = status;
    if (S.trace) {
        double* tr = S.trace + ((int64_t)b * S.n_lqr_iter + iter) * 5;
        tr[0] = mu_before; tr[1] = (double)acc; tr[2] = J_last; tr[3] = J_new; tr[4] = (double)n_eval;
    }
    if (status == DPILQR_STATUS_ACTIVE && S.next_items) {
        const int pos = atomicAdd(S.next_count, 1);
        S.next_items[pos] = b;
    }
    return acc;
}

template <int NS>
__device__ __forceinline__ double pair_cost_nd(const double* a, const double* b, int nd, double radius) {
    const double dx = a[0] - b[0], dy = a[1] - b[1];
    double s = 0.0;
    s += dx * dx;
    s += dy * dy;
    if (NS >= 3) {
        const double dz = a[2] - b[2];
        const double s3 = s + dz * dz;
        s = (nd >= 3) ? s3 : s;
    }
    if (nd < 2) s = dx * dx;
    if (s > radius * radius * (1.0 + 1e-12)) return 0.0;
    const double m = fmin(0.0, sqrt(s) - radius);
    return m * m;
}

template <int MODEL, int KA>
struct WaveFwdLds {
    static constexpr int NS = ModelDef<MODEL>::NS, NC = ModelDef<MODEL>::NC;
    static constexpr int n = KA * NS, m = KA * NC, NP = KA * (KA - 1) / 2, NP1 = NP > 0 ? NP : 1;
    static constexpr int LDG = (n % 4 == 0) ? n + 2 : n;
    static constexpr int NW = (KA * DPILQR_N_ALPHA + 63) / 64;
#ifndef DPILQR_LS_KGAP_ALL
#define DPILQR_LS_KGAP_ALL 0
#endif
#ifndef DPILQR_LS_NO_KGAP
#define DPILQR_LS_NO_KGAP 0
#endif
    static constexpr int kgap_for(int blk) { int g = 0; while ((((blk + g) / 2) & 1) == 0) g += 2; return g; }
    static constexpr int KBLK = NC * n;
    static constexpr int KGAP = (!DPILQR_LS_NO_KGAP && (NW > 1 || DPILQR_LS_KGAP_ALL) && KBLK % 2 == 0) ? kgap_for(KBLK) : 0;
    static constexpr int oK = 0;
    static constexpr int od = oK + m * n + KA * KGAP;
    static constexpr int odx = (od + m + 1) & ~1;
    static constexpr int oxs = odx + DPILQR_N_ALPHA * LDG;
    static constexpr int ocr = oxs + DPILQR_N_ALPHA * LDG;
    static constexpr int ocp = ocr + 2 * DPILQR_N_ALPHA * KA;
    static constexpr int oJ = ocp + 2 * DPILQR_N_ALPHA * NP1;
    static constexpr int IPB = NW == 1 ? 4 : 1;
    static constexpr int octl = oJ + DPILQR_N_ALPHA;
#ifndef DPILQR_LS_CL_ALL
#define DPILQR_LS_CL_ALL 0
#endif
    static constexpr bool CONST_LDS = NW > 1 || NS >= 6 || DPILQR_LS_CL_ALL;
#ifndef DPILQR_LS_OCC
#define DPILQR_LS_OCC 2
#endif
    static constexpr int OCC = ((NW > 1 && NS >= 6 && KA >= 9) || NS >= 12) ? 1 : DPILQR_LS_OCC;
#ifndef DPILQR_LS_PF
#define DPILQR_LS_PF 2
#endif
    static constexpr int PF = (NW == 1 && NS == 4 && !CONST_LDS) ? DPILQR_LS_PF : 1;
    static_assert(PF == 1 || PF == 2, "the horizon loop is written out for one or two register stages (step t, step t + 1)");
    static constexpr int oQ = (octl + 2 + 1) & ~1;
    static constexpr int oR = oQ + (CONST_LDS ? KA * NS * NS : 0);
    static constexpr int oXf = oR + (CONST_LDS ? KA * NC * NC : 0);
    static constexpr int total = (oXf + (CONST_LDS ? n : 0) + 1) & ~1;
};

template <int NW>
__device__ __forceinline__ void wave_sync() {
    if constexpr (NW == 1) asm volatile("" ::: "memory");
    else asm volatile("s_waitcnt lgkmcnt(0)\n\ts_barrier" ::: "memory");
}

template <int MODEL, int KA>
__global__ __launch_bounds__((64 * WaveFwdLds<MODEL, KA>::NW * WaveFwdLds<MODEL, KA>::IPB), (WaveFwdLds<MODEL, KA>::OCC)) void k_linesearch_wave(
    dpilqr_batch_desc D, double* X, double* U, const double* __restrict__ K, const double* __restrict__ d,
    const double* __restrict__ alphas, double* Xc, double* Uc, SolveState S, const int32_t* __restrict__ items,
    const int32_t* __restrict__ n_items) {
    using W = WaveFwdLds<MODEL, KA>;
    constexpr int NS = W::NS, NC = W::NC, n = W::n, m = W::m, mn = m * n, NPAIRS = W::NP, NP1 = W::NP1;
    constexpr int NG = DPILQR_N_ALPHA;
    constexpr int NW = W::NW, NTH = 64 * NW;
    constexpr int PPL = (NPAIRS + KA - 1) / KA;
    constexpr int KV = (mn / 2 + NTH - 1) / NTH;

    const int sub = NW == 1 ? __builtin_amdgcn_readfirstlane((int)(threadIdx.x >> 6)) : 0;
    const int tid = NW == 1 ? (int)(threadIdx.x & 63) : (int)threadIdx.x;
    const int slot = blockIdx.x * W::IPB + sub;
    if (slot >= *n_items) return;
    const int b = items[slot];
    const int T = D.T;
    extern __shared__ __attribute__((aligned(16))) double lds_all[];
    double* lds = lds_all + sub * W::total;
    double* Xb = X + (int64_t)b * (T + 1) * n;
    double* Ub = U + (int64_t)b * T * m;
    if (S.singular && S.singular[b]) {
        if (tid == 0) retire_without_gains(S, b);
        return;
    }
    const int64_t gslot = S.gains_by_item ? b : slot;
    const double* Kb = K + gslot * T * mn;
    const double* db = d + gslot * T * m;
    const bool active = tid < KA * NG;
    const int g = active ? tid / KA : 0, a = active ? tid - (tid / KA) * KA : 0;
    const double alpha = alphas[g];
    double* const Xw0 = Xc + (int64_t)slot * NG * (int64_t)(T + 1) * n;
    double* const Uw0 = Uc + (int64_t)slot * NG * (int64_t)T * m;
    int xw_off = g * (T + 1) * n + a * NS;
    asm volatile("" : "+v"(xw_off));
    auto uw_off_at = [&](int t_) {
        int g_ = g;
        asm volatile("" : "+v"(g_));
        return (unsigned)(g_ * (T * m) + a * NC + t_ * m);
    };

    const ItemParams P = item_params(D, b);
    constexpr bool CL = W::CONST_LDS;
    double xf_r[CL ? 1 : NS], Q_r[CL ? 1 : NS * NS], R_r[CL ? 1 : NC * NC];
    const double* xf = xf_r; const double* Q = Q_r; const double* R = R_r;
    if constexpr (CL) {
        for (int e = tid; e < KA * NS * NS; e += NTH) lds[W::oQ + e] = P.Q[e];
        for (int e = tid; e < KA * NC * NC; e += NTH) lds[W::oR + e] = P.R[e];
        for (int e = tid; e < n; e += NTH) lds[W::oXf + e] = P.xf[e];
        xf = lds + W::oXf + a * NS; Q = lds + W::oQ + a * NS * NS; R = lds + W::oR + a * NC * NC;
    } else {
#pragma unroll
        for (int i = 0; i < NS; ++i) xf_r[i] = P.xf[a * NS + i];
#pragma unroll
        for (int i = 0; i < NS * NS; ++i) Q_r[i] = P.Q[a * NS * NS + i];
#pragma unroll
        for (int i = 0; i < NC * NC; ++i) R_r[i] = P.R[a * NC * NC + i];
    }
    const double radius = P.radius;
    bool homog = true;
#pragma unroll
    for (int i = 1; i < KA; ++i) homog = homog && (P.n_dims[i] == P.n_dims[0]);
    int pp[PPL > 0 ? PPL : 1];
    auto make_pairs = [&](int a_) {
#pragma unroll
        for (int q = 0; q < PPL; ++q) {
            const int p = min(a_ + q * KA, NP1 - 1);
            int ii = 0, rem = p;
            while (rem >= KA - 1 - ii) { rem -= KA - 1 - ii; ++ii; }
            const int jj = ii + 1 + rem;
            pp[q] = ii | (jj << 8) | ((homog ? 2 : min(P.n_dims[ii], P.n_dims[jj])) << 16);
        }
    };
    make_pairs(a);

    double* sK = lds + W::oK;
    double* sd = lds + W::od;
    double* sdx = lds + W::odx + g * W::LDG;
    double* sxs = lds + W::oxs + g * W::LDG;
    double* scr0 = lds + W::ocr + g * KA;
    double* scp0 = lds + W::ocp + g * NP1;

    struct Stage { v2d stK[KV]; double std_, u[NC], xold[NS]; };
    constexpr int PF = W::PF;
    Stage stg[PF];
    double x[NS];
    auto fetch = [&](Stage& sg, int t) {
        const unsigned ko = (unsigned)(t * mn), xo = (unsigned)(t * n + a * NS), uo = (unsigned)(t * m + a * NC);
#ifdef DPILQR_LS_K_FIRST
#pragma unroll
        for (int q = 0; q < KV; ++q) {
            const int e = min(tid + NTH * q, mn / 2 - 1);
            sg.stK[q] = *reinterpret_cast<const v2d*>(Kb + (ko + 2u * (unsigned)e));
        }
#endif
#pragma unroll
        for (int i = 0; i < NS; ++i) sg.xold[i] = Xb[xo + (unsigned)i];
#pragma unroll
        for (int i = 0; i < NC; ++i) sg.u[i] = Ub[uo + (unsigned)i];
        sg.std_ = db[(unsigned)(t * m + min(tid, m - 1))];
#ifndef DPILQR_LS_K_FIRST
#pragma unroll
        for (int q = 0; q < KV; ++q) {
            const int e = min(tid + NTH * q, mn / 2 - 1);
            sg.stK[q] = *reinterpret_cast<const v2d*>(Kb + (ko + 2u * (unsigned)e));
        }
#endif
    };
    auto store_vec = [&](double* p, const double* v, int len) {
        if ((len & 1) == 0) {
#pragma unroll
            for (int i = 0; i < len; i += 2) store_v2d_nt(p + i, v2d{v[i], v[i + 1]});
        } else {
#pragma unroll
            for (int i = 0; i < len; ++i) store_f64_nt(p + i, v[i]);
        }
    };
    auto stage_cost = [&](double& J, int par) {
        const double* scp = scp0 + par * NG * NP1;
        const double* scr = scr0 + par * NG * KA;
        double prox = 0.0, ref = 0.0;
        if constexpr (NPAIRS > 32) {
            constexpr int CH = 8;
#pragma unroll 1
            for (int p0 = 0; p0 < NPAIRS; p0 += CH) {
                double v[CH];
#pragma unroll
                for (int q = 0; q < CH; ++q) v[q] = scp[min(p0 + q, NP1 - 1)];
#pragma unroll
                for (int q = 0; q < CH; ++q) prox = (p0 + q < NPAIRS) ? prox + v[q] : prox;
            }
        } else {
#pragma unroll
            for (int p = 0; p < NPAIRS; ++p) prox += scp[p];
        }
#pragma unroll
        for (int i = 0; i < KA; ++i) ref += scr[i];
        J += D.w_prox * prox + D.w_ref * ref;
    };
    auto post_costs = [&](double cr, const double* cp, int par) {
        if (active) {
            scr0[par * NG * KA + a] = cr;
#pragma unroll
            for (int q = 0; q < PPL; ++q)
                if (a + q * KA < NPAIRS) scp0[par * NG * NP1 + a + q * KA] = cp[q];
        }
    };

#pragma unroll
    for (int i = 0; i < NS; ++i) x[i] = Xb[a * NS + i];
#pragma unroll
    for (int s = 0; s < PF; ++s)
        if (s < T) fetch(stg[s], s);
    double J = 0.0;
    double ut[NC];
#pragma unroll
    for (int i = 0; i < NC; ++i) ut[i] = 0.0;

#ifdef DPILQR_PHASE_STAMPS
    unsigned long long w_wait = 0, w_t0 = __builtin_amdgcn_s_memtime();
#endif
    auto step = [&](Stage& sg, int t) {
        v2d (&stK)[KV] = sg.stK;
        double& std_ = sg.std_;
        double (&u)[NC] = sg.u;
        double (&xold)[NS] = sg.xold;
#ifdef DPILQR_PHASE_STAMPS
        {
            const unsigned long long a0 = __builtin_amdgcn_s_memtime();
            asm volatile("s_waitcnt vmcnt(0)" ::: "memory");
            w_wait += __builtin_amdgcn_s_memtime() - a0;
        }
#endif
#pragma unroll
        for (int q = 0; q < KV; ++q) {
            int tid_o = tid;
            if constexpr (W::KGAP > 0) asm volatile("" : "+v"(tid_o));
            const int e = min(tid_o + NTH * q, mn / 2 - 1);
            *reinterpret_cast<v2d*>(sK + 2 * e + (W::KGAP > 0 ? ((2 * e) / W::KBLK) * W::KGAP : 0)) = stK[q];
        }
        if (tid < m) sd[tid] = std_;
        if (active) {
            store_vec(Xw0 + (unsigned)(xw_off + t * n), x, NS);
            if (t > 0) store_vec(Uw0 + uw_off_at(t - 1), ut, NC);
        }
#pragma unroll
        for (int i = 0; i < NC; ++i) ut[i] = u[i];
        if (active) {
#pragma unroll
            for (int i = 0; i < NS; ++i) {
                sdx[a * NS + i] = x[i] - xold[i];
                sxs[a * NS + i] = x[i];
            }
        }
        wave_sync<NW>();
        if (t + PF < T) fetch(sg, t + PF);
        if (a == 0 && t > 0) stage_cost(J, (t & 1) ^ 1);
        DPILQR_LDS_FENCE();
        {
            double sum[NC];
#pragma unroll
            for (int c = 0; c < NC; ++c) sum[c] = 0.0;
            const double* rows = sK + a * (W::KBLK + W::KGAP);
            if (n % 2 == 0) {
#pragma unroll 5
                for (int j = 0; j < n; j += 2) {
                    const v2d dx2 = *reinterpret_cast<const v2d*>(lds + W::odx + g * W::LDG + j);
#pragma unroll
                    for (int c = 0; c < NC; ++c) {
                        const v2d kr = *reinterpret_cast<const v2d*>(rows + c * n + j);
                        sum[c] += kr.x * dx2.x;
                        sum[c] += kr.y * dx2.y;
                    }
                }
            } else {
#pragma unroll
                for (int j = 0; j < n; ++j) {
                    const double dxj = lds[W::odx + g * W::LDG + j];
#pragma unroll
                    for (int c = 0; c < NC; ++c) sum[c] += rows[c * n + j] * dxj;
                }
            }
#pragma unroll
            for (int c = 0; c < NC; ++c) {
                const double du = sum[c] + alpha * sd[a * NC + c];
                ut[c] = ut[c] + du;
            }
        }
        const double cr = ref_cost<NS, NC>(x, ut, xf, Q, R, false);
        double cp[PPL > 0 ? PPL : 1];
#pragma unroll
        for (int q = 0; q < PPL; ++q) cp[q] = pair_cost_nd<NS>(sxs + (pp[q] & 255) * NS, sxs + ((pp[q] >> 8) & 255) * NS, pp[q] >> 16, radius);
        DPILQR_LDS_FENCE();
        post_costs(cr, cp, t & 1);
        double xn[NS];
        integrate<MODEL>(x, ut, D.dt, xn);
#pragma unroll
        for (int i = 0; i < NS; ++i) x[i] = xn[i];
        wave_sync<NW>();
    };
    if constexpr (PF == 1) {
        for (int t = 0; t < T; ++t) step(stg[0], t);
    } else {
        int t = 0;
        for (; t + 1 < T; t += 2) { step(stg[0], t); step(stg[1], t + 1); }
        if (t < T) step(stg[0], t);
    }
#ifdef DPILQR_PHASE_STAMPS
    if (g_stamp_buf && tid == 0) {
        g_stamp_buf[2 * slot] = w_wait;
        g_stamp_buf[2 * slot + 1] = __builtin_amdgcn_s_memtime() - w_t0;
    }
#endif
    if (active) {
        store_vec(Xw0 + (unsigned)(xw_off + T * n), x, NS);
        if (T > 0) store_vec(Uw0 + uw_off_at(T - 1), ut, NC);
    }
    {
        if (active) {
#pragma unroll
            for (int i = 0; i < NS; ++i) sxs[a * NS + i] = x[i];
        }
        wave_sync<NW>();
        if (a == 0 && T > 0) stage_cost(J, (T & 1) ^ 1);
        if constexpr (NS >= 6 || NW > 1) {
            int a2 = a;
            asm volatile("" : "+v"(a2));
            make_pairs(a2);
        }
        double Qf[NS * NS], uz[NC];
#pragma unroll
        for (int i = 0; i < NS * NS; ++i) Qf[i] = P.Qf[a * NS * NS + i];
#pragma unroll
        for (int c = 0; c < NC; ++c) uz[c] = 0.0;
        const double cr = ref_cost<NS, NC>(x, uz, xf, Qf, R, true);
        double cp[PPL > 0 ? PPL : 1];
#pragma unroll
        for (int q = 0; q < PPL; ++q) cp[q] = pair_cost_nd<NS>(sxs + (pp[q] & 255) * NS, sxs + ((pp[q] >> 8) & 255) * NS, pp[q] >> 16, radius);
        DPILQR_LDS_FENCE();
        post_costs(cr, cp, T & 1);
        wave_sync<NW>();
        if (a == 0) stage_cost(J, T & 1);
    }
    if constexpr (NS >= 6 || NW > 1) {
        int tid2 = tid;
        asm volatile("" : "+v"(tid2));
        if (active && a == 0) lds[W::oJ + tid2 / KA] = J;
    } else {
        if (active && a == 0) lds[W::oJ + g] = J;
    }
    asm volatile("s_waitcnt vmcnt(0)" ::: "memory");
    __builtin_amdgcn_fence(__ATOMIC_ACQ_REL, "workgroup");
    wave_sync<NW>();
    int* ctl = reinterpret_cast<int*>(lds + W::octl);
    if (tid == 0) ctl[0] = linesearch_decide(S, b, NG, lds + W::oJ);
    __builtin_amdgcn_fence(__ATOMIC_ACQ_REL, "workgroup");
    wave_sync<NW>();
    const int acc = ctl[0];
    if (acc < 0) return;
    const double* Xa = Xc + ((int64_t)slot * NG + acc) * (int64_t)(T + 1) * n;
    const double* Ua = Uc + ((int64_t)slot * NG + acc) * (int64_t)T * m;
    for (int e = tid; e < (T + 1) * n; e += NTH) Xb[e] = Xa[e];
    for (int e = tid; e < T * m; e += NTH) Ub[e] = Ua[e];
}

template <int MODEL, int KA>
struct WaveRolloutLds {
    static constexpr int NS = ModelDef<MODEL>::NS, n = KA * NS, NP = KA * (KA - 1) / 2, NP1 = NP > 0 ? NP : 1;
    static constexpr int IPW = 64 / KA;
    static constexpr int oxs = 0, ocr = oxs + IPW * n, ocp = ocr + IPW * KA, total = (ocp + IPW * NP1 + 1) & ~1;
};

template <int MODEL, int KA>
__global__ __launch_bounds__(256) void k_rollout_wave(dpilqr_batch_desc D, const double* __restrict__ x0,
                                                      const double* __restrict__ U, double* __restrict__ X,
                                                      double* __restrict__ Jout) {
    using W = WaveRolloutLds<MODEL, KA>;
    constexpr int NS = W::NS, NC = ModelDef<MODEL>::NC, n = W::n, m = KA * NC, NPAIRS = W::NP, NP1 = W::NP1, IPW = W::IPW;
    constexpr PairTable<KA> PT{};
    constexpr int PPL = (NPAIRS + KA - 1) / KA;
    const int sub = __builtin_amdgcn_readfirstlane((int)(threadIdx.x >> 6));
    const int tid = threadIdx.x & 63;
    const bool lane_on = tid < IPW * KA;
    const int w = lane_on ? tid / KA : 0, a = lane_on ? tid - (tid / KA) * KA : 0;
    const int64_t b_raw = ((int64_t)blockIdx.x * 4 + sub) * IPW + w;
    const bool active = lane_on && b_raw < D.B;
    const int b = (int)(b_raw < D.B ? b_raw : D.B - 1);
    const int T = D.T;
    extern __shared__ __attribute__((aligned(16))) double lds_all[];
    double* lds = lds_all + sub * W::total;
    double* sxs = lds + W::oxs + w * n;
    double* scr = lds + W::ocr + w * KA;
    double* scp = lds + W::ocp + w * NP1;
    const ItemParams P = item_params(D, b);
    double xf[NS], Q[NS * NS], R[NC * NC];
#pragma unroll
    for (int i = 0; i < NS; ++i) xf[i] = P.xf[a * NS + i];
#pragma unroll
    for (int i = 0; i < NS * NS; ++i) Q[i] = P.Q[a * NS * NS + i];
#pragma unroll
    for (int i = 0; i < NC * NC; ++i) R[i] = P.R[a * NC * NC + i];
    const double radius = P.radius;
    bool homog = true;
#pragma unroll
    for (int i = 1; i < KA; ++i) homog = homog && (P.n_dims[i] == P.n_dims[0]);
    int pi[PPL > 0 ? PPL : 1], pj[PPL > 0 ? PPL : 1], pnd[PPL > 0 ? PPL : 1];
#pragma unroll
    for (int q = 0; q < PPL; ++q) {
        const int p = min(a + q * KA, NP1 - 1);
        int ii = 0, jj = 0;
#pragma unroll
        for (int e = 0; e < NPAIRS; ++e)
            if (e == p) { ii = PT.i[e]; jj = PT.j[e]; }
        pi[q] = ii; pj[q] = jj;
        pnd[q] = homog ? 2 : min(P.n_dims[ii], P.n_dims[jj]);
    }
    const double* Ub = U + (int64_t)b * T * m + a * NC;
    double* Xw = X + (int64_t)b * (T + 1) * n + a * NS;
    auto store_vec = [&](double* p, const double* v, int len) {
        if ((len & 1) == 0) {
#pragma unroll
            for (int i = 0; i < len; i += 2) store_v2d_nt(p + i, v2d{v[i], v[i + 1]});
        } else {
#pragma unroll
            for (int i = 0; i < len; ++i) store_f64_nt(p + i, v[i]);
        }
    };
    auto stage_cost = [&](double& J) {
        double prox = 0.0, ref = 0.0;
#pragma unroll
        for (int p = 0; p < NPAIRS; ++p) prox += scp[p];
#pragma unroll
        for (int i = 0; i < KA; ++i) ref += scr[i];
        J += D.w_prox * prox + D.w_ref * ref;
    };
    double x[NS], u[NC], un[NC];
#pragma unroll
    for (int i = 0; i < NS; ++i) x[i] = x0[(int64_t)b * n + a * NS + i];
#pragma unroll
    for (int i = 0; i < NC; ++i) un[i] = (T > 0) ? Ub[i] : 0.0;
    double J = 0.0;
    for (int t = 0; t < T; ++t) {
        if (active) store_vec(Xw + (int64_t)t * n, x, NS);
#pragma unroll
        for (int i = 0; i < NC; ++i) u[i] = un[i];
        if (t + 1 < T) {
#pragma unroll
            for (int i = 0; i < NC; ++i) un[i] = Ub[(int64_t)(t + 1) * m + i];
        }
#pragma unroll
        for (int i = 0; i < NS; ++i) sxs[a * NS + i] = x[i];
        DPILQR_LDS_FENCE();
        if (a == 0 && t > 0) stage_cost(J);
        const double cr = ref_cost<NS, NC>(x, u, xf, Q, R, false);
        double cp[PPL > 0 ? PPL : 1];
#pragma unroll
        for (int q = 0; q < PPL; ++q) cp[q] = pair_cost_nd<NS>(sxs + pi[q] * NS, sxs + pj[q] * NS, pnd[q], radius);
        DPILQR_LDS_FENCE();
        scr[a] = cr;
#pragma unroll
        for (int q = 0; q < PPL; ++q)
            if (a + q * KA < NPAIRS) scp[a + q * KA] = cp[q];
        double xn[NS];
        integrate<MODEL>(x, u, D.dt, xn);
#pragma unroll
        for (int i = 0; i < NS; ++i) x[i] = xn[i];
    }
    if (active) store_vec(Xw + (int64_t)T * n, x, NS);
#pragma unroll
    for (int i = 0; i < NS; ++i) sxs[a * NS + i] = x[i];
    DPILQR_LDS_FENCE();
    if (a == 0 && T > 0) stage_cost(J);
    {
        double Qf[NS * NS], uz[NC];
#pragma unroll
        for (int i = 0; i < NS * NS; ++i) Qf[i] = P.Qf[a * NS * NS + i];
#pragma unroll
        for (int c = 0; c < NC; ++c) uz[c] = 0.0;
        const double cr = ref_cost<NS, NC>(x, uz, xf, Qf, R, true);
        double cp[PPL > 0 ? PPL : 1];
#pragma unroll
        for (int q = 0; q < PPL; ++q) cp[q] = pair_cost_nd<NS>(sxs + pi[q] * NS, sxs + pj[q] * NS, pnd[q], radius);
        DPILQR_LDS_FENCE();
        scr[a] = cr;
#pragma unroll
        for (int q = 0; q < PPL; ++q)
            if (a + q * KA < NPAIRS) scp[a + q * KA] = cp[q];
        DPILQR_LDS_FENCE();
        if (a == 0) stage_cost(J);
    }
    if (active && a == 0) Jout[b] = J;
}

}
```

### dpilqr_amd/csrc/launch.hpp

```cpp
#pragma once
#include <hip/hip_runtime.h>

#include <cstdint>
#include <cstdlib>

#include "dpilqr_hip.h"
#include "solve_state.hpp"

namespace dpilqr {

int32_t fail(int32_t code, const char* fmt, ...);
const char* last_error();

#define HIP_TRY(expr)                                                                                 \
    do {                                                                                              \
        hipError_t e_ = (expr);                                                                       \
        if (e_ != hipSuccess) return ::dpilqr::fail(DPILQR_EHIP, "%s failed: %s", #expr, hipGetErrorString(e_)); \
    } while (0)

constexpr int kMaxLds = 160 * 1024;

template <typename Kern>
inline int32_t allow_lds(Kern kern, size_t bytes) {
    if (bytes > (size_t)kMaxLds) return fail(DPILQR_EUNSUPPORTED, "needs %zu B of LDS per workgroup (> %d)", bytes, kMaxLds);
    if (bytes > 64 * 1024)
        HIP_TRY(hipFuncSetAttribute(reinterpret_cast<const void*>(kern), hipFuncAttributeMaxDynamicSharedMemorySize, (int)bytes));
    return DPILQR_OK;
}

#define DISPATCH_FAMILY_CASE(NS_, NC_, ...) case NS_: { constexpr int NS = NS_, NC = NC_; __VA_ARGS__ } break;
#define DISPATCH_FAMILY_CASES(ns, ...)                                                    \
    DISPATCH_FAMILY_CASE(3, 2, __VA_ARGS__)                                               \
    DISPATCH_FAMILY_CASE(4, 2, __VA_ARGS__)                                               \
    DISPATCH_FAMILY_CASE(6, 3, __VA_ARGS__)                                               \
    DISPATCH_FAMILY_CASE(12, 4, __VA_ARGS__)                                              \
    default: return ::dpilqr::fail(DPILQR_EINVAL, "unsupported per-agent state dim %d", (int)(ns));
#define DISPATCH_FAMILY(ns, BODY) switch (ns) { DISPATCH_FAMILY_CASES(ns, BODY) }
#define DISPATCH_FAMILY_ALL(ns, BODY) switch (ns) { DISPATCH_FAMILY_CASE(5, 2, BODY) DISPATCH_FAMILY_CASES(ns, BODY) }

int device_cus();

const char* route_env(const char* name);
inline bool route_flag(const char* name) { return route_env(name) != nullptr; }
inline int route_int(const char* name, int dflt) { const char* e = route_env(name); return (e && *e) ? atoi(e) : dflt; }

inline int hint_model(const dpilqr_batch_desc& D) { return (D.uniform_model & 0xff) - 1; }
inline int hint_n_dims(const dpilqr_batch_desc& D) { return ((D.uniform_model >> 8) & 0xff) - 1; }
inline bool hint_shared_weights(const dpilqr_batch_desc& D) { return ((D.uniform_model >> 16) & 1) != 0; }
inline bool hint_planar4(const dpilqr_batch_desc& D) { return ((D.uniform_model >> 17) & 1) != 0 || hint_model(D) == 0 || hint_model(D) == 3; }
inline bool fused_wavefront_sweep_applies(const dpilqr_batch_desc& D) {
    static const bool off = route_flag("DPILQR_NO_FUSED");
    return !off && hint_model(D) == 0 && hint_n_dims(D) == 2 && hint_shared_weights(D) && D.Q_bstride == 0 && D.R_bstride == 0 &&
           D.Qf_bstride == 0 && D.n_s == 4 && D.n_c == 2 && D.k <= 5;
}
inline bool fused_wavefront_general_applies(const dpilqr_batch_desc& D) {
    static const bool off = route_flag("DPILQR_NO_FUSED") || route_flag("DPILQR_NO_FUSED_GENERAL");
    return !off && hint_planar4(D) && hint_n_dims(D) == 2 && D.n_s == 4 && D.n_c == 2 && D.k <= 5;
}
inline bool fused_workgroup_sweep_applies(const dpilqr_batch_desc& D) {
    static const bool off = route_flag("DPILQR_NO_FUSED") || route_flag("DPILQR_NO_FUSED_WG");
    return !off && ((D.n_s == 4 && D.n_c == 2 && D.k >= 6 && D.k <= 15) || (D.n_s == 6 && D.n_c == 3 && D.k >= 2 && D.k <= 10));
}
inline bool fused_wavefront_inprod_applies(const dpilqr_batch_desc& D) {
    static const bool off = route_flag("DPILQR_NO_FUSED") || route_flag("DPILQR_NO_INPROD");
    static const bool no4 = route_flag("DPILQR_NO_INPROD4");
    if (off) return false;
    if (D.n_s == 4 && D.n_c == 2 && D.k <= 5 && !no4)
        return !fused_wavefront_sweep_applies(D) && !fused_wavefront_general_applies(D);
    return (D.n_s == 6 && D.n_c == 3 && D.k <= 4) || (D.n_s == 3 && D.n_c == 2 && D.k <= 6) || (D.n_s == 5 && D.n_c == 2 && D.k <= 4);
}
inline bool fused_sweep_applies(const dpilqr_batch_desc& D) {
    return fused_wavefront_sweep_applies(D) || fused_wavefront_general_applies(D) || fused_workgroup_sweep_applies(D) ||
           fused_wavefront_inprod_applies(D);
}
inline bool solve_prefers_records(const dpilqr_batch_desc& D) {
    static const bool off = route_flag("DPILQR_NO_WAVE_PREF");
    if (fused_wavefront_inprod_applies(D)) {
        static const bool rec = route_flag("DPILQR_INPROD_RECORDS");
        return rec || (!off && D.n_s == 5 && D.k <= 2);
    }
    return !off && ((D.n_s == 6 && D.n_c == 3 && (D.k == 2 || D.k == 3 || D.k == 4)) || (D.n_s == 4 && D.n_c == 2 && D.k == 6));
}

int32_t launch_make_tiles(const dpilqr_batch_desc& D, const double* X, const double* U, double* tiles,
                          const int32_t* items, const int32_t* n_items, int grid_items, bool sparse, bool dyn_only,
                          hipStream_t st);
int32_t tile_layout_host(int32_t n_x, int32_t n_u, int64_t offsets[7], int64_t row_strides[7], int64_t* stride);

extern thread_local int g_sweep_waves;
int32_t launch_riccati(int B, int T, int n, int m, const double* tiles, const double* mu, double* K, double* d,
                       int32_t* singular, const int32_t* items, const int32_t* n_items, int grid_items,
                       int gains_by_item, int block_ns, int block_nc, hipStream_t st);
int32_t launch_riccati_fused(const dpilqr_batch_desc& D, const double* X, const double* U, const double* mu, double* K,
                             double* d, int32_t* singular, const int32_t* items, const int32_t* n_items, int grid_items,
                             int gains_by_item, hipStream_t st);
int32_t set_stamp_buffer_riccati(void* device_buffer);

constexpr int sweep_waves(int grid_items, int max_wv, size_t lds_per_wave, bool tier12) {
    return (tier12 && grid_items > 2048 && max_wv >= 12 && lds_per_wave * 12 <= (size_t)kMaxLds) ? 12
           : (grid_items > 1024 && max_wv >= 8 && lds_per_wave * 8 <= (size_t)kMaxLds) ? 8 : 4;
}
constexpr int sweep_grid(int grid_items, int cus, int wv) {
    return grid_items <= cus ? grid_items : (grid_items + cus * wv - 1) / (cus * wv) * cus;
}
inline int sweep_max_waves() { static const int v = route_int("DPILQR_MFMA_WAVES", 12); return v; }
template <typename Kern, typename... Args>
int32_t launch_sweep_kernel(Kern kern, int wv, int threads, size_t lds, int grid_items, int cus, hipStream_t st, const Args&... args) {
    const int32_t rc = allow_lds(kern, lds);
    if (rc) return rc;
    hipLaunchKernelGGL(kern, dim3(sweep_grid(grid_items, cus, wv)), dim3(threads), lds, st, args...);
    HIP_TRY(hipGetLastError());
    g_sweep_waves = wv;
    return DPILQR_OK;
}
template <typename T> struct same_type { using type = T; };
template <typename Kern, typename... Args>
int32_t launch_wave_sweep(Kern k4, typename same_type<Kern>::type k8, typename same_type<Kern>::type k12, size_t lds_per_wave,
                          int grid_items, int cus, hipStream_t st, const Args&... args) {
    const int wv = sweep_waves(grid_items, sweep_max_waves(), lds_per_wave, k12 != nullptr);
    return launch_sweep_kernel(wv == 12 ? k12 : (wv == 8 ? k8 : k4), wv, 64 * wv, lds_per_wave * wv, grid_items, cus, st, args...);
}
int32_t launch_riccati_team(const dpilqr_batch_desc& D, const double* X, const double* U, const double* mu, double* K, double* d,
                            int32_t* singular, const int32_t* items, const int32_t* n_items, int grid_items, int gains_by_item,
                            hipStream_t st);

int32_t launch_riccati_inprod(const dpilqr_batch_desc& D, const double* X, const double* U, const double* mu, double* K, double* d,
                              int32_t* singular, const int32_t* items, const int32_t* n_items, int grid_items, int gains_by_item,
                              hipStream_t st);

int32_t launch_riccati_bike(const dpilqr_batch_desc& D, const double* X, const double* U, const double* mu, double* K, double* d,
                            int32_t* singular, const int32_t* items, const int32_t* n_items, int grid_items, int gains_by_item,
                            hipStream_t st);

int fused_sweep_tier(const dpilqr_batch_desc& D, int grid_items);
int32_t launch_cost_keys(const dpilqr_batch_desc& D, const double* X, const int32_t* list, const int32_t* count, int grid_items,
                         int min_live, int32_t* key, int32_t* key_dense, hipStream_t st);
int32_t launch_order_list(const int32_t* src, int32_t* dst, const int32_t* count, const int32_t* key, int T, int cus, int waves,
                          int order, int min_live, hipStream_t st);

int32_t launch_linesearch_team(const dpilqr_batch_desc& D, double* X, double* U, const double* K, const double* d,
                               const double* alphas, double* Xc, double* Uc, const SolveState& S, const int32_t* items,
                               const int32_t* n_items, int grid_items, hipStream_t st);

int32_t launch_forward(const dpilqr_batch_desc& D, int mode, const double* x0, double* X, double* U, const double* K,
                       const double* d, const double* alphas, int ngrp, double* Xc, double* Uc, double* Jc,
                       const SolveState& S, const int32_t* items, const int32_t* n_items, int grid_items,
                       hipStream_t st);
int32_t set_stamp_buffer_forward(void* device_buffer);
int32_t launch_model_op(int op, int32_t n, int32_t ns, const int32_t* model, const double* x, const double* u, double dt,
                        double* o1, double* o2, hipStream_t st);
int32_t launch_cost_eval(const dpilqr_batch_desc& D, int32_t n_pts, const double* x, const double* u, int32_t terminal,
                         double* cost, hipStream_t st);
int32_t launch_pairwise_graph(int32_t S, int32_t N, int32_t k, int32_t n_s, const double* X, const double* radius,
                              int32_t* adj, hipStream_t st);


constexpr int kRouteSmallMaxNx = 60, kRouteSmallMaxK = 20, kRouteLargeMaxNx = 240, kRouteLargeMaxK = 20;

struct PolicyPlan {
    const double *X, *U, *K;
    int32_t kc_max;
    const uint64_t* nbr_bits;
};
struct PolicyRolloutArgs {
    PolicyPlan plan;
    int32_t n_samples;
    const double *x0s, *W, *u_lim;
    double *Xs, *Us, *J, *min_sep, *goal_dist;
};
struct PolicyAdvanceArgs {
    PolicyPlan plan;
    int32_t h;
    const int32_t* scen;
    int32_t n_scen, L, n_d;
    const double *W, *u_lim;
    double* x_cur;
    int32_t* n_done;
    double *X_exec, *U_exec, *J_exec, *min_sep, *dist_left, *U_next, *X_next;
};
inline int32_t check_kc_max(const char* who, const dpilqr_batch_desc& D, int32_t kc_max) {
    return kc_max >= 1 && kc_max <= D.k ? DPILQR_OK
                                        : fail(DPILQR_EUNSUPPORTED, "%s: kc_max=%d, a neighbourhood has 1 .. k = %d members", who, kc_max, D.k);
}

int32_t launch_policy_rollout(const dpilqr_batch_desc& D, const PolicyRolloutArgs& a, hipStream_t st);
int32_t launch_policy_rollout_dec(const dpilqr_batch_desc& D, const PolicyRolloutArgs& a, hipStream_t st);
int32_t launch_policy_rollout_dec_team(const dpilqr_batch_desc& D, const PolicyRolloutArgs& a, hipStream_t st);
int32_t launch_policy_rollout_dec_wide(const dpilqr_batch_desc& D, const PolicyRolloutArgs& a, int32_t n_words, hipStream_t st);
int32_t launch_policy_rollout_large(const dpilqr_batch_desc& D, const PolicyRolloutArgs& a, hipStream_t st);
int32_t launch_policy_advance(const dpilqr_batch_desc& D, const PolicyAdvanceArgs& a, hipStream_t st);
int32_t launch_policy_advance_dec_team(const dpilqr_batch_desc& D, const PolicyAdvanceArgs& a, hipStream_t st);
int32_t launch_policy_advance_dec_wide(const dpilqr_batch_desc& D, const PolicyAdvanceArgs& a, int32_t n_words, hipStream_t st);
int32_t launch_policy_advance_large(const dpilqr_batch_desc& D, const PolicyAdvanceArgs& a, hipStream_t st);

int32_t launch_rollout_wide(const dpilqr_batch_desc& D, const double* x0, const double* U, double* X, double* J, double* min_sep,
                            double* goal_dist, hipStream_t st);

int64_t riccati_big_scratch_elems(int n, int m);
int32_t launch_riccati_big_f64(const dpilqr_batch_desc& D, const double* X, const double* U, const double* mu, double* K,
                               double* d, int32_t* singular, const int32_t* items, const int32_t* n_items,
                               int grid_items, int gains_by_item, void* scratch, hipStream_t st);
int32_t launch_riccati_big_f32(const dpilqr_batch_desc& D, const float* X, const float* U, const double* mu, float* K,
                               float* d, int32_t* singular, const int32_t* items, const int32_t* n_items,
                               int grid_items, int gains_by_item, void* scratch, hipStream_t st);
int32_t launch_forward_big_f64(const dpilqr_batch_desc& D, int mode, const double* x0, double* X, double* U, const double* K,
                               const double* d, const double* alphas, int ngrp, double* Xc, double* Uc, double* Jc,
                               const SolveState& S, const int32_t* items, const int32_t* n_items, int grid_items,
                               hipStream_t st);
int32_t launch_forward_big_f32(const dpilqr_batch_desc& D, int mode, const float* x0, float* X, float* U, const float* K,
                               const float* d, const double* alphas, int ngrp, float* Xc, float* Uc, double* Jc,
                               const SolveState& S, const int32_t* items, const int32_t* n_items, int grid_items,
                               hipStream_t st);
inline bool uses_big_path(int n_x) {
    static const bool force = route_flag("DPILQR_FORCE_BIG");
    return force || n_x > 60;
}

}
```

### dpilqr_amd/csrc/solve_state.hpp

```cpp
#pragma once
#include <cstdint>

#include "dpilqr_hip.h"

namespace dpilqr {

enum ForwardMode : int { kModeRollout = 0, kModeCandidates = 1, kModeLineSearch = 2 };

struct SolveState {
    double* mu;
    double* delta;
    double* J_star;
    double* J_last;
    int32_t* status;
    int32_t* n_bwd;
    int32_t* n_fwd;
    double* trace;
    const int32_t* singular;
    int32_t* fault;
    int32_t* next_count;
    int32_t* next_items;
    int32_t n_lqr_iter;
    int32_t gains_by_item;
    double tol;
    const int64_t* t_admit;
    int64_t t_kill_ticks;
};

__device__ inline bool solve_time_is_up(const SolveState& S, int b) {
    if (S.t_kill_ticks <= 0) return false;
    return (int64_t)__builtin_amdgcn_s_memrealtime() - S.t_admit[b] > S.t_kill_ticks;
}

__device__ inline void retire_without_gains(const SolveState& S, int b) {
    const bool fault = S.singular[b] == 2;
    S.status[b] = fault ? DPILQR_STATUS_FAULT : DPILQR_STATUS_SINGULAR;
    S.n_bwd[b] += 1;
    if (fault && S.fault) atomicAdd(S.fault, 1);
}

}
```

### dpilqr_amd/csrc/tu_forward.hip

```cpp
#include <hip/hip_runtime.h>

#include <cstdlib>

#include "launch.hpp"
#include "forward.hpp"
#include "forward_wave.hpp"

namespace dpilqr {

static int forward_threads(int k, int ngrp) {
    const int t = ((k * ngrp + 63) / 64) * 64;
    return t;
}

static bool no_wave_ro() { static const bool v = route_flag("DPILQR_FORWARD_GENERIC"); return v; }

int32_t launch_forward(const dpilqr_batch_desc& D, int mode, const double* x0, double* X, double* U, const double* K,
                       const double* d, const double* alphas, int ngrp, double* Xc, double* Uc, double* Jc,
                       const SolveState& S, const int32_t* items, const int32_t* n_items, int grid_items,
                       hipStream_t st) {
    if (grid_items <= 0) return DPILQR_OK;
    const int n = D.k * D.n_s, m = D.k * D.n_c;
    int threads = forward_threads(D.k, mode == kModeRollout ? 1 : ngrp);
    if (threads > 256) return fail(DPILQR_EUNSUPPORTED, "k*n_alpha=%d exceeds the 256-thread workgroup of the forward pass", D.k * ngrp);
    const size_t lds_item = (forward_lds_bytes(n, m, D.k, ngrp) + 15) & ~(size_t)15;
    if (uses_big_path(n) || lds_item > (size_t)kMaxLds || (mode != kModeRollout && (m * n + threads - 1) / threads > kMaxStage))
        return launch_forward_big_f64(D, mode, x0, X, U, K, d, alphas, ngrp, Xc, Uc, Jc, S, items, n_items, grid_items, st);
    if (!no_wave_ro() && mode == kModeRollout && hint_model(D) >= 0 && !items) {
        const int model = hint_model(D);
#define DPILQR_TRY_RO(MODEL, KA)                                                                                    \
    if (model == MODEL && D.k == KA && model_ns(MODEL) == D.n_s && model_nc(MODEL) == D.n_c) {                      \
        using WR = WaveRolloutLds<MODEL, KA>;                                                                       \
        const int per_wg = 4 * WR::IPW;                                                                             \
        hipLaunchKernelGGL((k_rollout_wave<MODEL, KA>), dim3((grid_items + per_wg - 1) / per_wg), dim3(256),        \
                           sizeof(double) * WR::total * 4, st, D, x0, U, X, Jc);                                    \
        HIP_TRY(hipGetLastError());                                                                                 \
        return DPILQR_OK;                                                                                           \
    }
#define DPILQR_RO_10(MODEL) DPILQR_TRY_RO(MODEL, 1) DPILQR_TRY_RO(MODEL, 2) DPILQR_TRY_RO(MODEL, 3)                \
        DPILQR_TRY_RO(MODEL, 4) DPILQR_TRY_RO(MODEL, 5) DPILQR_TRY_RO(MODEL, 6) DPILQR_TRY_RO(MODEL, 7)             \
        DPILQR_TRY_RO(MODEL, 8) DPILQR_TRY_RO(MODEL, 9) DPILQR_TRY_RO(MODEL, 10)
#define DPILQR_RO_15(MODEL) DPILQR_RO_10(MODEL) DPILQR_TRY_RO(MODEL, 11) DPILQR_TRY_RO(MODEL, 12)                   \
        DPILQR_TRY_RO(MODEL, 13) DPILQR_TRY_RO(MODEL, 14) DPILQR_TRY_RO(MODEL, 15)
        DPILQR_RO_15(kDoubleInt4D)
        DPILQR_RO_15(kUnicycle4D)
        DPILQR_RO_10(kQuadcopter6D)
#define DPILQR_RO_6(MODEL) DPILQR_TRY_RO(MODEL, 1) DPILQR_TRY_RO(MODEL, 2) DPILQR_TRY_RO(MODEL, 3)                 \
        DPILQR_TRY_RO(MODEL, 4) DPILQR_TRY_RO(MODEL, 5) DPILQR_TRY_RO(MODEL, 6)
        DPILQR_RO_6(kDoubleInt6D)
        DPILQR_RO_6(kCar3D)
        DPILQR_RO_6(kBike5D)
        DPILQR_RO_6(kHuman6D)
        DPILQR_RO_6(kHumanLin6D)
        DPILQR_TRY_RO(kQuadcopter12D, 1) DPILQR_TRY_RO(kQuadcopter12D, 2) DPILQR_TRY_RO(kQuadcopter12D, 3)
        DPILQR_TRY_RO(kQuadcopter12D, 4) DPILQR_TRY_RO(kQuadcopter12D, 5)
#undef DPILQR_RO_6
#undef DPILQR_RO_15
#undef DPILQR_RO_10
#undef DPILQR_TRY_RO
    }
    static const bool no_wave = route_flag("DPILQR_FORWARD_GENERIC");
    if (!no_wave && mode == kModeLineSearch && hint_model(D) >= 0 && ngrp == DPILQR_N_ALPHA && items && n_items) {
        const int model = hint_model(D);
        {
            const int32_t rc_t = launch_linesearch_team(D, X, U, K, d, alphas, Xc, Uc, S, items, n_items, grid_items, st);
            if (rc_t != DPILQR_EUNSUPPORTED) return rc_t;
        }
#define DPILQR_TRY_WAVE(MODEL, KA)                                                                                  \
    if (model == MODEL && D.k == KA && model_ns(MODEL) == D.n_s && model_nc(MODEL) == D.n_c) {                      \
        using WF = WaveFwdLds<MODEL, KA>;                                                                           \
        const size_t lds_w = sizeof(double) * WF::total * WF::IPB;                                                  \
        int32_t rc_w = allow_lds(k_linesearch_wave<MODEL, KA>, lds_w);                                              \
        if (rc_w) return rc_w;                                                                                      \
        hipLaunchKernelGGL((k_linesearch_wave<MODEL, KA>), dim3((grid_items + WF::IPB - 1) / WF::IPB),              \
                           dim3(64 * WF::NW * WF::IPB), lds_w, st, D, X, U, K, d, alphas, Xc, Uc, S, items, n_items); \
        HIP_TRY(hipGetLastError());                                                                                 \
        return DPILQR_OK;                                                                                           \
    }
#define DPILQR_WAVE_10(MODEL) DPILQR_TRY_WAVE(MODEL, 1) DPILQR_TRY_WAVE(MODEL, 2) DPILQR_TRY_WAVE(MODEL, 3)        \
        DPILQR_TRY_WAVE(MODEL, 4) DPILQR_TRY_WAVE(MODEL, 5) DPILQR_TRY_WAVE(MODEL, 6) DPILQR_TRY_WAVE(MODEL, 7)     \
        DPILQR_TRY_WAVE(MODEL, 8) DPILQR_TRY_WAVE(MODEL, 9) DPILQR_TRY_WAVE(MODEL, 10)
#define DPILQR_WAVE_15(MODEL) DPILQR_WAVE_10(MODEL) DPILQR_TRY_WAVE(MODEL, 11) DPILQR_TRY_WAVE(MODEL, 12)           \
        DPILQR_TRY_WAVE(MODEL, 13) DPILQR_TRY_WAVE(MODEL, 14) DPILQR_TRY_WAVE(MODEL, 15)
        DPILQR_WAVE_15(kDoubleInt4D)
        DPILQR_WAVE_15(kUnicycle4D)
        DPILQR_WAVE_10(kQuadcopter6D)
#define DPILQR_WAVE_6(MODEL) DPILQR_TRY_WAVE(MODEL, 1) DPILQR_TRY_WAVE(MODEL, 2) DPILQR_TRY_WAVE(MODEL, 3)         \
        DPILQR_TRY_WAVE(MODEL, 4) DPILQR_TRY_WAVE(MODEL, 5) DPILQR_TRY_WAVE(MODEL, 6)
        DPILQR_WAVE_6(kDoubleInt6D)
        DPILQR_WAVE_6(kCar3D)
        DPILQR_WAVE_6(kBike5D)
        DPILQR_WAVE_6(kHuman6D)
        DPILQR_WAVE_6(kHumanLin6D)
        DPILQR_TRY_WAVE(kQuadcopter12D, 1) DPILQR_TRY_WAVE(kQuadcopter12D, 2) DPILQR_TRY_WAVE(kQuadcopter12D, 3)
        DPILQR_TRY_WAVE(kQuadcopter12D, 4)
#undef DPILQR_WAVE_6
#undef DPILQR_WAVE_15
#undef DPILQR_WAVE_10
#undef DPILQR_TRY_WAVE
    }
    static const bool no_pack = route_flag("DPILQR_FORWARD_NO_PACK");
    const int ipb = (!no_pack && threads == 64 && 4 * lds_item <= (size_t)kMaxLds) ? 4 : 1;
    const size_t lds = lds_item * ipb;
    threads *= ipb;
    DISPATCH_FAMILY_ALL(D.n_s, {
        int32_t rc = allow_lds(k_forward<double, NS, NC, false>, lds);
        if (rc) return rc;
        hipLaunchKernelGGL((k_forward<double, NS, NC, false>), dim3((grid_items + ipb - 1) / ipb), dim3(threads), lds, st, D, mode,
                           x0, X, U, K, d, alphas, ngrp, Xc, Uc, Jc, S, items, n_items, ipb, (int)(lds_item / sizeof(double)));
    })
    HIP_TRY(hipGetLastError());
    return DPILQR_OK;
}

int32_t set_stamp_buffer_forward(void* buf) {
    void* p = buf;
    HIP_TRY(hipMemcpyToSymbol(HIP_SYMBOL(g_stamp_buf), &p, sizeof(p)));
    return DPILQR_OK;
}

int32_t launch_model_op(int op, int32_t n, int32_t ns, const int32_t* model, const double* x, const double* u, double dt,
                        double* o1, double* o2, hipStream_t st) {
    const dim3 grid((n + 63) / 64), block(64);
    DISPATCH_FAMILY_ALL(ns, {
        if (op == 0) hipLaunchKernelGGL((k_model_op<NS, NC, 0>), grid, block, 0, st, n, model, x, u, dt, o1, o2);
        else if (op == 1) hipLaunchKernelGGL((k_model_op<NS, NC, 1>), grid, block, 0, st, n, model, x, u, dt, o1, o2);
        else hipLaunchKernelGGL((k_model_op<NS, NC, 2>), grid, block, 0, st, n, model, x, u, dt, o1, o2);
    })
    HIP_TRY(hipGetLastError());
    return DPILQR_OK;
}

int32_t launch_cost_eval(const dpilqr_batch_desc& D, int32_t n_pts, const double* x, const double* u, int32_t terminal,
                         double* cost, hipStream_t st) {
    const int64_t total = (int64_t)D.B * n_pts;
    const dim3 grid((unsigned)((total + 63) / 64)), block(64);
    DISPATCH_FAMILY_ALL(D.n_s, {
        hipLaunchKernelGGL((k_cost_eval<NS, NC>), grid, block, 0, st, D, n_pts, x, u, terminal, cost);
    })
    HIP_TRY(hipGetLastError());
    return DPILQR_OK;
}

int32_t launch_pairwise_graph(int32_t S, int32_t N, int32_t k, int32_t n_s, const double* X, const double* radius,
                              int32_t* adj, hipStream_t st) {
    HIP_TRY(hipMemsetAsync(adj, 0, sizeof(int32_t) * (size_t)S * k * k, st));
    const int64_t total = (int64_t)S * (k * (k - 1) / 2 + k);
    hipLaunchKernelGGL(k_pairwise_graph, dim3((unsigned)((total + 127) / 128)), dim3(128), 0, st, S, N, k, n_s, X, radius, adj);
    HIP_TRY(hipGetLastError());
    return DPILQR_OK;
}

}
```

### dpilqr_amd/csrc/tu_lsteam.hip

```cpp
#include <hip/hip_runtime.h>

#include <cstdlib>

#include "launch.hpp"
#include "forward_team.hpp"

namespace dpilqr {

int32_t launch_linesearch_team(const dpilqr_batch_desc& D, double* X, double* U, const double* K, const double* d,
                               const double* alphas, double* Xc, double* Uc, const SolveState& S, const int32_t* items,
                               const int32_t* n_items, int grid_items, hipStream_t st) {
    static const bool off = route_flag("DPILQR_LS_NO_TEAM");
    static const int max_items = route_int("DPILQR_LS_TEAM_MAX", 1024);
    if (off || grid_items > max_items || grid_items <= 0 || hint_model(D) < 0) return DPILQR_EUNSUPPORTED;
    const int model = hint_model(D);
#define DPILQR_TRY_LSTEAM(MODEL, KA)                                                                                \
    if (model == MODEL && D.k == KA && model_ns(MODEL) == D.n_s && model_nc(MODEL) == D.n_c) {                      \
        using TF = TeamFwdLds<MODEL, KA>;                                                                           \
        const size_t lds_t = sizeof(double) * TF::total;                                                            \
        hipLaunchKernelGGL((k_linesearch_team<MODEL, KA>), dim3(grid_items), dim3(128), lds_t, st, D, X, U, K, d,   \
                           alphas, Xc, Uc, S, items, n_items);                                                      \
        HIP_TRY(hipGetLastError());                                                                                 \
        return DPILQR_OK;                                                                                           \
    }
#define DPILQR_LSTEAM_6(MODEL) DPILQR_TRY_LSTEAM(MODEL, 1) DPILQR_TRY_LSTEAM(MODEL, 2) DPILQR_TRY_LSTEAM(MODEL, 3) \
        DPILQR_TRY_LSTEAM(MODEL, 4) DPILQR_TRY_LSTEAM(MODEL, 5) DPILQR_TRY_LSTEAM(MODEL, 6)
    DPILQR_LSTEAM_6(kDoubleInt4D)
    DPILQR_LSTEAM_6(kUnicycle4D)
    DPILQR_LSTEAM_6(kQuadcopter6D)
    DPILQR_LSTEAM_6(kDoubleInt6D)
    DPILQR_LSTEAM_6(kCar3D)
#undef DPILQR_LSTEAM_6
#undef DPILQR_TRY_LSTEAM
    return DPILQR_EUNSUPPORTED;
}

}
```

### dpilqr_amd/csrc/tu_order.hip

```cpp
#include <hip/hip_runtime.h>

#define DPILQR_ADMIT_ORDER_KERNELS
#include "admit_order.hpp"
#include "launch.hpp"
#include "riccati_mfma.hpp"

namespace dpilqr {

int fused_sweep_tier(const dpilqr_batch_desc& D, int grid_items) {
    if (!fused_wavefront_sweep_applies(D) || grid_items <= kOrderMinLive) return 0;
    const int n = D.k * D.n_s, m = D.k * D.n_c;
#define DPILQR_TIER(NN, MM) \
    if (n == NN && m == MM) return sweep_waves(grid_items, sweep_max_waves(), sizeof(double) * MfmaCfg<NN, MM, true>::total, true);
    DPILQR_TIER(4, 2) DPILQR_TIER(8, 4) DPILQR_TIER(12, 6) DPILQR_TIER(16, 8) DPILQR_TIER(20, 10)
#undef DPILQR_TIER
    return 0;
}

int32_t launch_cost_keys(const dpilqr_batch_desc& D, const double* X, const int32_t* list, const int32_t* count, int grid_items,
                         int min_live, int32_t* key, int32_t* key_dense, hipStream_t st) {
    if (grid_items <= 0) return DPILQR_OK;
    hipLaunchKernelGGL(k_cost_keys, dim3((grid_items + 3) / 4), dim3(256), 0, st, X, D.radius, D.radius_bstride, list, count, D.B, D.T,
                       D.k, min_live, key, key_dense);
    HIP_TRY(hipGetLastError());
    return DPILQR_OK;
}

int32_t launch_order_list(const int32_t* src, int32_t* dst, const int32_t* count, const int32_t* key, int T, int cus, int waves,
                          int order, int min_live, hipStream_t st) {
    hipLaunchKernelGGL(k_order_list, dim3(1), dim3(1024), 0, st, src, dst, count, key, T, cus, waves, order, min_live);
    HIP_TRY(hipGetLastError());
    return DPILQR_OK;
}

}
```

### include/dpilqr_hip.h

```cpp
#ifndef DPILQR_HIP_H
#define DPILQR_HIP_H

#include <stdint.h>

#ifdef __cplusplus
extern "C" {
#endif

#define DPILQR_ABI_VERSION 4

#define DPILQR_OK 0
#define DPILQR_EINVAL (-1)
#define DPILQR_EUNSUPPORTED (-2)
#define DPILQR_EHIP (-3)
#define DPILQR_ENOGPU (-4)
#define DPILQR_EWORKSPACE (-5)

#define DPILQR_MODEL_DOUBLE_INT_4D 0
#define DPILQR_MODEL_DOUBLE_INT_6D 1
#define DPILQR_MODEL_CAR_3D 2
#define DPILQR_MODEL_UNICYCLE_4D 3
#define DPILQR_MODEL_QUADCOPTER_6D 4
#define DPILQR_MODEL_HUMAN_6D 5
#define DPILQR_MODEL_HUMAN_LIN_6D 6
#define DPILQR_MODEL_QUADCOPTER_12D 7
#define DPILQR_MODEL_HUMAN_PAD_12D 8
#define DPILQR_MODEL_BIKE_5D 10

#define DPILQR_STATUS_ACTIVE 0
#define DPILQR_STATUS_CONVERGED 1
#define DPILQR_STATUS_LINESEARCH_FAILED 2
#define DPILQR_STATUS_MAX_ITER 3
#define DPILQR_STATUS_SINGULAR 4
#define DPILQR_STATUS_KILLED 5
#define DPILQR_STATUS_FAULT 6

#define DPILQR_N_ALPHA 10

typedef struct dpilqr_batch_desc {
    int32_t B;
    int32_t k;
    int32_t n_s;
    int32_t n_c;
    int32_t T;
    int32_t uniform_model;
    double dt;
    double w_ref;
    double w_prox;
    const int32_t* model;  int64_t model_bstride;
    const int32_t* n_dims; int64_t n_dims_bstride;
    const double* xf;      int64_t xf_bstride;
    const double* Q;       int64_t Q_bstride;
    const double* R;       int64_t R_bstride;
    const double* Qf;      int64_t Qf_bstride;
    const double* radius;  int64_t radius_bstride;
} dpilqr_batch_desc;

int32_t dpilqr_abi_version(void);
const char* dpilqr_last_error(void);
int32_t dpilqr_device_info(int32_t dev, int32_t* n_cu, int32_t* lds_bytes, char* arch, int32_t arch_len);
int32_t dpilqr_model_dims(int32_t model, int32_t* n_s, int32_t* n_c);

int32_t dpilqr_model_f(int32_t n, int32_t family_ns, const int32_t* model, const double* x, const double* u,
                       double* x_dot, void* stream);
int32_t dpilqr_model_integrate(int32_t n, int32_t family_ns, const int32_t* model, const double* x,
                               const double* u, double dt, double* x_new, void* stream);
int32_t dpilqr_model_linearize(int32_t n, int32_t family_ns, const int32_t* model, const double* x,
                               const double* u, double dt, double* A ,
                               double* B , void* stream);

int32_t dpilqr_cost_eval(const dpilqr_batch_desc* desc, int32_t n_pts, const double* x, const double* u,
                         int32_t terminal, double* cost , void* stream);

int32_t dpilqr_tile_layout(int32_t n_x, int32_t n_u, int64_t offsets[7], int64_t row_strides[7], int64_t* stride);
int32_t dpilqr_make_tiles(const dpilqr_batch_desc* desc, const double* X, const double* U, double* tiles,
                          const int32_t* items, const int32_t* n_items, void* stream);

int32_t dpilqr_rollout(const dpilqr_batch_desc* desc, const double* x0, const double* U, double* X, double* J,
                       void* stream);
int32_t dpilqr_backward_pass_tiles(int32_t B, int32_t T, int32_t n_x, int32_t n_u, const double* tiles,
                                   const double* mu, double* K, double* d, int32_t* singular,
                                   const int32_t* items, const int32_t* n_items, void* stream);
int32_t dpilqr_backward_pass_tiles_blocks(int32_t B, int32_t T, int32_t n_x, int32_t n_u, int32_t block_ns,
                                          int32_t block_nc, const double* tiles, const double* mu, double* K,
                                          double* d, int32_t* singular, const int32_t* items,
                                          const int32_t* n_items, void* stream);
int64_t dpilqr_tiles_bytes(int32_t B, int32_t T, int32_t n_x, int32_t n_u);
int32_t dpilqr_backward_pass(const dpilqr_batch_desc* desc, const double* X, const double* U, const double* mu,
                             double* K, double* d, double* tiles_workspace, void* stream);
int32_t dpilqr_backward_pass_fused(const dpilqr_batch_desc* desc, const double* X, const double* U, const double* mu, double* K,
                                   double* d, int32_t* singular, void* stream);
int32_t dpilqr_forward_pass(const dpilqr_batch_desc* desc, const double* X, const double* U, const double* K,
                            const double* d, const double* alphas, int32_t n_alpha, double* Xn, double* Un,
                            double* Jn, void* stream);

int32_t dpilqr_alphas(double* alphas_host);

int64_t dpilqr_solve_workspace_bytes(const dpilqr_batch_desc* desc, int32_t window, int32_t gains_in_workspace);
typedef struct dpilqr_solver dpilqr_solver;
int32_t dpilqr_solver_create(dpilqr_solver** out);
int32_t dpilqr_solver_destroy(dpilqr_solver* solver);
typedef void (*dpilqr_progress_fn)(void* user, int32_t n_finished, int32_t n_items);
int32_t dpilqr_solver_set_progress(dpilqr_solver* solver, dpilqr_progress_fn fn, void* user);
int32_t dpilqr_solve_batch(dpilqr_solver* solver, const dpilqr_batch_desc* desc, const double* x0, double* U,
                           int32_t n_lqr_iter, double tol, double t_kill, int32_t window, void* workspace, int64_t workspace_bytes,
                           double* X, double* J, int32_t* status, int32_t* n_bwd, int32_t* n_fwd, double* trace,
                           double* K_out, double* d_out, void* stream);
int32_t dpilqr_solve_enqueue(const dpilqr_batch_desc* desc, const double* x0, double* U, int32_t n_lqr_iter, double tol,
                             double t_kill, int32_t window, void* workspace, int64_t workspace_bytes, double* X, double* J,
                             int32_t* status, int32_t* n_bwd, int32_t* n_fwd, double* trace, double* K_out,
                             double* d_out, int32_t n_global_iter, int32_t resume, void* stream);
int64_t dpilqr_solve_iterations_bound(const dpilqr_batch_desc* desc, int32_t window, int32_t n_lqr_iter);

int32_t dpilqr_rollout_f32(const dpilqr_batch_desc* desc, const float* x0, const float* U, float* X, double* J, void* stream);
int64_t dpilqr_backward_pass_workspace_bytes(const dpilqr_batch_desc* desc, int32_t elem_bytes );
int32_t dpilqr_backward_pass_f32(const dpilqr_batch_desc* desc, const float* X, const float* U, const double* mu, float* K,
                                 float* d, void* workspace, void* stream);
int32_t dpilqr_forward_pass_f32(const dpilqr_batch_desc* desc, const float* X, const float* U, const float* K, const float* d,
                                const double* alphas, int32_t n_alpha, float* Xn, float* Un, double* Jn, void* stream);
int64_t dpilqr_solve_workspace_bytes_f32(const dpilqr_batch_desc* desc, int32_t window, int32_t gains_in_workspace);
int32_t dpilqr_solve_batch_f32(dpilqr_solver* solver, const dpilqr_batch_desc* desc, const float* x0, float* U,
                               int32_t n_lqr_iter, double tol, double t_kill, int32_t window, void* workspace, int64_t workspace_bytes,
                               float* X, double* J, int32_t* status, int32_t* n_bwd, int32_t* n_fwd, double* trace,
                               float* K_out, float* d_out, void* stream);

int32_t dpilqr_profile_enable(dpilqr_solver* solver , int32_t enable);
int32_t dpilqr_debug_stamps(void* device_buffer);
int32_t dpilqr_profile_read(dpilqr_solver* solver, double ms[4], int64_t launches[4], int64_t items[4], int32_t reset);
int32_t dpilqr_profile_read_sweep(dpilqr_solver* solver, int32_t waves, double* ms, int64_t* launches, int64_t* items, int32_t reset);

int32_t dpilqr_pairwise_graph(int32_t S, int32_t N, int32_t k, int32_t n_s, const double* X,
                              const double* radius , int32_t* adj, void* stream);

#define DPILQR_MAX_AGENTS 64
typedef struct dpilqr_bucket_results {
    const double* X[DPILQR_MAX_AGENTS + 1];
    const double* U[DPILQR_MAX_AGENTS + 1];
    int32_t first[DPILQR_MAX_AGENTS + 1];
    int32_t count[DPILQR_MAX_AGENTS + 1];
} dpilqr_bucket_results;
int32_t dpilqr_dispatch_graph(int32_t S, int32_t N, int32_t k, int32_t n_s, const double* X, const double* radius,
                              int64_t radius_stride, const int32_t* ignore, uint64_t* bits, int32_t* rep, int32_t* size,
                              int32_t* order, int32_t* slot, int32_t* bucket_start, int32_t* bucket_count, void* stream);
int32_t dpilqr_dispatch_gather(int32_t k, int32_t n_s, int32_t n_c, int32_t T, int32_t n_rows, int32_t kc, const int32_t* order,
                               int32_t first, int32_t count, const uint64_t* bits, const double* X, const double* U,
                               const double* xf, int64_t xf_stride, double* x0_out, double* xf_out, double* U_out,
                               int32_t* members, void* stream);
int32_t dpilqr_dispatch_gather_params(int32_t count, int32_t kc, int32_t width, int32_t elem_bytes, const int32_t* members,
                                      const void* src, void* out, void* stream);
int32_t dpilqr_dispatch_stitch(int32_t S, int32_t k, int32_t n_s, int32_t n_c, int32_t T, const uint64_t* bits, const int32_t* rep,
                               const int32_t* size, const int32_t* slot, const dpilqr_bucket_results* results, double* X_dec,
                               double* U_dec, void* stream);
int32_t dpilqr_dispatch_pack_rows(int32_t S, int32_t k, int32_t n_s, int32_t n_c, int32_t T, const uint64_t* bits,
                                  const int32_t* rep, const int32_t* size, const int32_t* slot,
                                  const dpilqr_bucket_results* results, int32_t* row_of, int32_t* n_rows, double* rows,
                                  int64_t row_len, void* stream);
int32_t dpilqr_dispatch_scatter_rows(int64_t n_rows_total, int32_t k, int32_t n_s, int32_t n_c, int32_t T, const double* rows,
                                     int64_t row_len, double* X_dec, double* U_dec, void* stream);

int32_t dpilqr_random_setup(int32_t S, int64_t seed0, int32_t k, int32_t n_s, int32_t n_d, double var, double energy,
                            double* x0, double* xf, void* stream);

#include "dpilqr_policy.h"
#include "dpilqr_swarm.h"
#include "dpilqr_swarm_policy.h"
#include "dpilqr_swarm_advance.h"
#include "dpilqr_swarm_study.h"
#include "dpilqr_order.h"
#include "dpilqr_nearest.h"
#include "dpilqr_separated_setup.h"

#ifdef __cplusplus
}
#endif
#endif
```

Before: 1.032 million subproblems/s.

## Emit cost-order keys from forward pass and fuse admit with ordering

The rollout and line-search wave kernels now record per-item near-collision keys as a side product of the pair-cost evaluation and store them in a new per-item workspace region. When those keys are fresh, one fused single-block admit+order kernel replaces the separate admit, cost-keys and order-list launches each iteration. This removes a pass over the trajectories plus two launches per iteration, at the cost of extra work and registers inside the forward kernels and new consistency checks between the forward path and the ordering path.

```diff
diff --git a/dpilqr_amd/_lib.py b/dpilqr_amd/_lib.py
--- a/dpilqr_amd/_lib.py
+++ b/dpilqr_amd/_lib.py
@@ -115,6 +115,12 @@
 }
 ORDER_SPREAD, ORDER_GROUPED = 1, 2
 
+LOOP_KEYS_SIGNATURES = {
+    "dpilqr_solve_item_keys_offset": (i64, [_DP, i32, i32]),
+    "dpilqr_admit": (i32, [vp, vp, vp, vp, i32, i32, vp, i32, vp, vp, vp]),
+    "dpilqr_admit_order": (i32, [vp, vp, vp, vp, i32, i32, vp, i32, vp, vp, vp, i32, i32, i32, i32, i32, vp, vp]),
+}
+
 _GW = SWARM_SIGNATURES["dpilqr_dispatch_graph_wide"][1]
 NEAREST_SIGNATURES = {"dpilqr_dispatch_graph_nearest": (i32, _GW[:8] + [i32] + _GW[8:15] + [vp] + _GW[15:])}
 
@@ -153,7 +159,7 @@
                               "(hipcc --offload-arch=gfx950).  dpilqr_amd has no CPU fallback.")
         lib = C.CDLL(str(LIB_PATH))
         for name, (res, args) in {**SIGNATURES, **EXT_SIGNATURES, **SWARM_SIGNATURES, **SWARM_POLICY_SIGNATURES, **SWARM_ADVANCE_SIGNATURES,
-                                   **ORDER_SIGNATURES, **NEAREST_SIGNATURES, **SWARM_STUDY_SIGNATURES, **SEPARATED_SIGNATURES}.items():
+                                   **ORDER_SIGNATURES, **LOOP_KEYS_SIGNATURES, **NEAREST_SIGNATURES, **SWARM_STUDY_SIGNATURES, **SEPARATED_SIGNATURES}.items():
             fn = getattr(lib, name)
             fn.restype = res
             fn.argtypes = args
diff --git a/dpilqr_amd/csrc/admit_order.hpp b/dpilqr_amd/csrc/admit_order.hpp
--- a/dpilqr_amd/csrc/admit_order.hpp
+++ b/dpilqr_amd/csrc/admit_order.hpp
@@ -63,6 +63,31 @@
     const int c = top < kOrderClasses ? key : (int)((int64_t)key * (kOrderClasses - 1) / top);
     return c < 0 ? 0 : (c > kOrderClasses - 1 ? kOrderClasses - 1 : c);
 }
+
+#if defined(__HIPCC__)
+
+__device__ inline int admit_items(int32_t* list, int base, int first, int B, int window, bool want_prefix, int64_t* t_admit,
+                                  int* lowest, int* prefix) {
+    const int n_new = min(B - first, window - base);
+    if (threadIdx.x == 0) *lowest = first;
+    __syncthreads();
+    for (int i = threadIdx.x; i < n_new; i += blockDim.x) list[base + i] = first + i;
+    if (t_admit && n_new > 0) {
+        const int64_t now = (int64_t)__builtin_amdgcn_s_memrealtime();
+        for (int i = threadIdx.x; i < n_new; i += blockDim.x) t_admit[first + i] = now;
+    }
+    if (want_prefix) {
+        int lo = first;
+        for (int i = threadIdx.x; i < base; i += blockDim.x) lo = min(lo, list[i]);
+        for (int off = 32; off > 0; off >>= 1) lo = min(lo, __shfl_down(lo, off));
+        if ((threadIdx.x & 63) == 0) atomicMin(lowest, lo);
+        __syncthreads();
+    }
+    *prefix = want_prefix ? *lowest : 0;
+    return n_new;
+}
+
+#endif
 
 #if defined(__HIPCC__) && defined(DPILQR_ADMIT_ORDER_KERNELS)
 
@@ -157,6 +182,48 @@
     }
 }
 
+__global__ void __launch_bounds__(1024) k_admit_order(int32_t* list, int32_t* __restrict__ dst, int32_t* count, int32_t* next_count,
+                                                      int32_t* admitted, int B, int window, int32_t* mail, int want_prefix,
+                                                      int64_t* t_admit, const int32_t* fault, const int32_t* __restrict__ item_key,
+                                                      int T, int n_cus, int waves, int order, int min_live) {
+    static_assert(kOrderClasses == 64, "the prefix sums below are one wavefront's, a bin per lane");
+    __shared__ int hist[kOrderClasses], cursor[kOrderClasses], lowest;
+    const int base = *count, first = *admitted;
+    int prefix;
+    const int n_new = admit_items(list, base, first, B, window, mail && want_prefix, t_admit, &lowest, &prefix);
+    const int n = base + n_new;
+    if (threadIdx.x < kOrderClasses) hist[threadIdx.x] = 0;
+    __syncthreads();
+    auto bin_of = [&](int b) { return kOrderClasses - 1 - order_class((b >= 0 && b < B) ? item_key[b] : 0, T); };
+    if (n <= min_live || order == kOrderOff) {
+        for (int i = threadIdx.x; i < n; i += blockDim.x) dst[i] = list[i];
+    } else {
+        for (int i = threadIdx.x; i < n; i += blockDim.x) atomicAdd(&hist[bin_of(list[i])], 1);
+        __syncthreads();
+        if (threadIdx.x < kOrderClasses) {
+            const int own = hist[threadIdx.x];
+            int run = own;
+            for (int off = 1; off < kOrderClasses; off <<= 1) {
+                const int below = __shfl_up(run, off);
+                if ((int)threadIdx.x >= off) run += below;
+            }
+            cursor[threadIdx.x] = run - own;
+        }
+        __syncthreads();
+        const SweepDeal deal(n, n_cus, waves);
+        for (int i = threadIdx.x; i < n; i += blockDim.x) {
+            const int b = list[i];
+            const int rank = atomicAdd(&cursor[bin_of(b)], 1);
+            const int pos = order_position(rank, deal, order);
+            if (pos >= 0 && pos < n) dst[pos] = b;
+        }
+    }
+    if (threadIdx.x == 0) {
+        *count = n; *admitted = first + n_new; *next_count = 0;
+        if (mail) { mail[0] = n; mail[1] = first + n_new; mail[2] = prefix; mail[3] = *fault; }
+    }
+}
+
 #endif
 
 }
diff --git a/dpilqr_amd/csrc/dpilqr_hip.hip b/dpilqr_amd/csrc/dpilqr_hip.hip
--- a/dpilqr_amd/csrc/dpilqr_hip.hip
+++ b/dpilqr_amd/csrc/dpilqr_hip.hip
@@ -108,25 +108,12 @@
 __global__ void k_admit(int32_t* list, int32_t* count, int32_t* next_count, int32_t* admitted, int B, int window,
                         int32_t* mail, int want_prefix, int64_t* t_admit, const int32_t* fault) {
     const int base = *count, first = *admitted;
-    const int n_new = min(B - first, window - base);
     __shared__ int lowest;
-    if (threadIdx.x == 0) lowest = first;
-    __syncthreads();
-    for (int i = threadIdx.x; i < n_new; i += blockDim.x) list[base + i] = first + i;
-    if (t_admit && n_new > 0) {
-        const int64_t now = (int64_t)__builtin_amdgcn_s_memrealtime();
-        for (int i = threadIdx.x; i < n_new; i += blockDim.x) t_admit[first + i] = now;
-    }
-    if (mail && want_prefix) {
-        int lo = first;
-        for (int i = threadIdx.x; i < base; i += blockDim.x) lo = min(lo, list[i]);
-        for (int off = 32; off > 0; off >>= 1) lo = min(lo, __shfl_down(lo, off));
-        if ((threadIdx.x & 63) == 0) atomicMin(&lowest, lo);
-        __syncthreads();
-    }
+    int prefix;
+    const int n_new = admit_items(list, base, first, B, window, mail && want_prefix, t_admit, &lowest, &prefix);
     if (threadIdx.x == 0) {
         *count = base + n_new; *admitted = first + n_new; *next_count = 0;
-        if (mail) { mail[0] = base + n_new; mail[1] = first + n_new; mail[2] = want_prefix ? lowest : 0; mail[3] = *fault; }
+        if (mail) { mail[0] = base + n_new; mail[1] = first + n_new; mail[2] = prefix; mail[3] = *fault; }
     }
 }
 
@@ -149,7 +136,7 @@
 };
 
 struct SolveWorkspace {
-    size_t tiles, K, d, Xc, Uc, mu, delta, J_star, J_last, alphas, singular, lists, counts, t_admit, total;
+    size_t tiles, K, d, Xc, Uc, mu, delta, J_star, J_last, alphas, singular, lists, counts, t_admit, item_keys, total;
     SolveWorkspace(const dpilqr_batch_desc& D, int W, bool gains_in_ws, SolveShape sh) {
         const size_t B = D.B, n = (size_t)D.k * D.n_s, m = (size_t)D.k * D.n_c, T = D.T, Wn = W, e = sh.elem;
         const TileLayout L((int)n, (int)m);
@@ -170,6 +157,7 @@
         lists = o;    o = al(o + sizeof(int32_t) * 2 * Wn);
         counts = o;   o = al(o + sizeof(int32_t) * (kCountRing + 2));
         t_admit = o;  o = al(o + sizeof(int64_t) * B);
+        item_keys = o; o = al(o + sizeof(int32_t) * 2 * B);
         total = o;
     }
 };
@@ -400,6 +388,23 @@
     const bool fused = sh.fused;
     const bool static_part = !fused && !sh.big && !no_static && D.R_bstride == 0 &&
                              (um == kDoubleInt4D || um == kDoubleInt6D || um == kHumanLin6D);
+    static const bool keys_kernel_route = route_flag("DPILQR_LOOP_KEYS_KERNEL");
+    static const int order_route = route_flag("DPILQR_NO_COST_ORDER") ? (int)kOrderOff : route_int("DPILQR_COST_ORDER", kDefaultCostOrder);
+    static const bool dense_key = !route_flag("DPILQR_NO_DECOUPLED") && route_int("DPILQR_COST_KEY", kDefaultCostKey) == (int)kKeyDenseSteps;
+    const int order = (sizeof(R) == 8 && fused && (order_route == kOrderSpread || order_route == kOrderGrouped)) ? order_route : (int)kOrderOff;
+    int32_t* keys = reinterpret_cast<int32_t*>(ws + W.Xc);
+    int32_t* item_keys = reinterpret_cast<int32_t*>(ws + W.item_keys);
+    const bool loop_keys = sizeof(R) == 8 && order != kOrderOff && !keys_kernel_route && fused_wavefront_sweep_applies(D) &&
+                           forward_emits_keys(D, kModeRollout, D.B);
+    if (loop_keys) { S.key_count = item_keys; S.key_dense = item_keys + D.B; }
+    auto wrote_keys = [&](int mode, int grid, bool* fresh) -> int32_t {
+        *fresh = loop_keys && forward_emits_keys(D, mode, grid);
+        if (sizeof(R) == 8 && *fresh != (loop_keys && g_forward_keys))
+            return fail(DPILQR_EHIP, "solve_batch: the forward pass (mode %d, %d items) %s the cost-order keys", mode, grid,
+                        *fresh ? "did not write" : "wrote");
+        return DPILQR_OK;
+    };
+    bool keys_fresh = loop_keys && resume && forward_emits_keys(D, kModeLineSearch, Wn);
     if (!resume) {
         double a[DPILQR_N_ALPHA];
         alpha_table(a);
@@ -412,6 +417,7 @@
                                 nullptr, D.B, st);
         if (rc) return bail(rc);
         prof.end(st);
+        if ((rc = wrote_keys(kModeRollout, D.B, &keys_fresh))) return bail(rc);
         hipLaunchKernelGGL(k_copy_f64, dim3((D.B + 255) / 256), dim3(256), 0, st, D.B, S.J_star, S.J_last);
         if (n_lqr_iter > 0) {
             if (!fused && hipMemsetAsync(tiles, 0, W.K - W.tiles, st) != hipSuccess) return bail(fail(DPILQR_EHIP, "hipMemsetAsync failed"));
@@ -423,10 +429,6 @@
         }
     }
 
-    static const int order_route = route_flag("DPILQR_NO_COST_ORDER") ? (int)kOrderOff : route_int("DPILQR_COST_ORDER", kDefaultCostOrder);
-    static const bool dense_key = !route_flag("DPILQR_NO_DECOUPLED") && route_int("DPILQR_COST_KEY", kDefaultCostKey) == (int)kKeyDenseSteps;
-    const int order = (sizeof(R) == 8 && fused && (order_route == kOrderSpread || order_route == kOrderGrouped)) ? order_route : (int)kOrderOff;
-    int32_t* keys = reinterpret_cast<int32_t*>(ws + W.Xc);
     int surv = 0;
     size_t n_iterations = 0;
     auto enqueue_iteration = [&](int it, int upper) -> int32_t {
@@ -435,15 +437,24 @@
         int32_t* cur_n = counts + (it % kCountRing);
         int32_t* nxt_n = counts + ((it + 1) % kCountRing);
         int32_t* mail = solver ? solver->dev + kMailWords * (it % kMailRing) : nullptr;
-        hipLaunchKernelGGL(k_admit, dim3(1), dim3(256), 0, st, cur, cur_n, nxt_n, admitted_dev, D.B, Wn, mail,
-                           (solver && solver->progress) ? 1 : 0, t_admit, S.fault);
-        if (solver) HIP_TRY(hipEventRecord(solver->ev[it % kMailRing], st));
+        const int want_prefix = (solver && solver->progress) ? 1 : 0;
         int32_t r = DPILQR_OK;
         const int order_waves = order ? fused_sweep_tier(D, upper) : 0;
+        if (order_waves > 0 && keys_fresh) {
+            if ((r = launch_admit_order(cur, other, cur_n, nxt_n, admitted_dev, D.B, Wn, mail, want_prefix, t_admit, S.fault,
+                                        dense_key ? S.key_dense : S.key_count, D.T, device_cus(), order_waves, order, kOrderMinLive, st)))
+                return r;
+        } else {
+            hipLaunchKernelGGL(k_admit, dim3(1), dim3(256), 0, st, cur, cur_n, nxt_n, admitted_dev, D.B, Wn, mail, want_prefix, t_admit,
+                               S.fault);
+        }
+        if (solver) HIP_TRY(hipEventRecord(solver->ev[it % kMailRing], st));
         if (order_waves > 0) {
             if constexpr (sizeof(R) == 8) {
-                if ((r = launch_cost_keys(D, X, cur, cur_n, upper, kOrderMinLive, dense_key ? nullptr : keys, dense_key ? keys : nullptr, st))) return r;
-                if ((r = launch_order_list(cur, other, cur_n, keys, D.T, device_cus(), order_waves, order, kOrderMinLive, st))) return r;
+                if (!keys_fresh) {
+                    if ((r = launch_cost_keys(D, X, cur, cur_n, upper, kOrderMinLive, dense_key ? nullptr : keys, dense_key ? keys : nullptr, st))) return r;
+                    if ((r = launch_order_list(cur, other, cur_n, keys, D.T, device_cus(), order_waves, order, kOrderMinLive, st))) return r;
+                }
             }
             S.next_items = cur;
             cur = other;
@@ -479,7 +490,7 @@
                                     upper, st)))
             return r;
         prof.end(st);
-        return DPILQR_OK;
+        return wrote_keys(kModeLineSearch, upper, &keys_fresh);
     };
 
     if (n_lqr_iter > 0 && solver) {
@@ -978,6 +989,40 @@
     return launch_order_list(items, out, n_items, keys, T, n_cus, waves, order, -1, as_stream(stream));
 }
 
+int64_t dpilqr_solve_item_keys_offset(const dpilqr_batch_desc* desc, int32_t window, int32_t gains_in_workspace) {
+    if (!desc || desc->B < 0 || desc->k < 1 || desc->T < 1) return fail(DPILQR_EINVAL, "solve_item_keys_offset: bad desc");
+    return (int64_t)SolveWorkspace(*desc, window_of(*desc, window), gains_in_workspace != 0, shape_of<double>(*desc)).item_keys;
+}
+
+static int32_t check_admit(const char* who, const int32_t* list, const int32_t* count, const int32_t* next_count, const int32_t* admitted,
+                           int32_t B, int32_t window, const int32_t* mail, const int32_t* fault) {
+    if (!list || !count || !next_count || !admitted || (mail && !fault)) return fail(DPILQR_EINVAL, "%s: NULL pointer", who);
+    if (B < 0 || window < 1) return fail(DPILQR_EINVAL, "%s: B=%d window=%d", who, B, window);
+    return DPILQR_OK;
+}
+
+int32_t dpilqr_admit(int32_t* list, int32_t* count, int32_t* next_count, int32_t* admitted, int32_t B, int32_t window, int32_t* mail,
+                     int32_t want_prefix, int64_t* t_admit, const int32_t* fault, void* stream) {
+    const int32_t rc = check_admit("admit", list, count, next_count, admitted, B, window, mail, fault);
+    if (rc) return rc;
+    hipLaunchKernelGGL(k_admit, dim3(1), dim3(256), 0, as_stream(stream), list, count, next_count, admitted, B, window, mail, want_prefix,
+                       t_admit, fault);
+    HIP_TRY(hipGetLastError());
+    return DPILQR_OK;
+}
+
+int32_t dpilqr_admit_order(int32_t* list, int32_t* count, int32_t* next_count, int32_t* admitted, int32_t B, int32_t window, int32_t* mail,
+                           int32_t want_prefix, int64_t* t_admit, const int32_t* fault, const int32_t* item_keys, int32_t T,
+                           int32_t n_cus, int32_t waves, int32_t order, int32_t min_live, int32_t* out, void* stream) {
+    const int32_t rc = check_admit("admit_order", list, count, next_count, admitted, B, window, mail, fault);
+    if (rc) return rc;
+    if (!item_keys || !out) return fail(DPILQR_EINVAL, "admit_order: NULL pointer");
+    if (T < 1 || n_cus < 1 || (waves != 4 && waves != 8 && waves != 12) || (order != kOrderSpread && order != kOrderGrouped))
+        return fail(DPILQR_EINVAL, "admit_order: T=%d n_cus=%d waves=%d order=%d", T, n_cus, waves, order);
+    return launch_admit_order(list, out, count, next_count, admitted, B, window, mail, want_prefix, t_admit, fault, item_keys, T, n_cus,
+                              waves, order, min_live, as_stream(stream));
+}
+
 int32_t dpilqr_order_position(int32_t rank, int32_t n, int32_t n_cus, int32_t waves, int32_t order) {
     if (n < 1 || rank < 0 || rank >= n || n_cus < 1 || (waves != 4 && waves != 8 && waves != 12) ||
         (order != kOrderSpread && order != kOrderGrouped))
diff --git a/dpilqr_amd/csrc/forward_wave.hpp b/dpilqr_amd/csrc/forward_wave.hpp
--- a/dpilqr_amd/csrc/forward_wave.hpp
+++ b/dpilqr_amd/csrc/forward_wave.hpp
@@ -56,7 +56,7 @@
 }
 
 template <int NS>
-__device__ __forceinline__ double pair_cost_nd(const double* a, const double* b, int nd, double radius) {
+__device__ __forceinline__ double pair_cost_nd(const double* a, const double* b, int nd, double radius, bool& near) {
     const double dx = a[0] - b[0], dy = a[1] - b[1];
     double s = 0.0;
     s += dx * dx;
@@ -67,9 +67,29 @@
         s = (nd >= 3) ? s3 : s;
     }
     if (nd < 2) s = dx * dx;
-    if (s > radius * radius * (1.0 + 1e-12)) return 0.0;
+    const bool far = s > radius * radius * (1.0 + 1e-12);
+    near = !far;
+    if (far) return 0.0;
     const double m = fmin(0.0, sqrt(s) - radius);
     return m * m;
+}
+template <int NS>
+__device__ __forceinline__ double pair_cost_nd(const double* a, const double* b, int nd, double radius) {
+    bool near;
+    return pair_cost_nd<NS>(a, b, nd, radius, near);
+}
+
+constexpr int kWaveKeySteps = 64;
+template <int MODEL, int KA>
+constexpr bool wave_emits_keys = MODEL == 0 && KA <= 5;
+__device__ __forceinline__ void wave_key_step(unsigned long long& bits, bool near) { bits = (bits << 1) | (near ? 1ull : 0ull); }
+template <int KA>
+__device__ __forceinline__ void wave_key_combine(unsigned long long bits, int first, int T, int& count, int& dense) {
+    unsigned long long any = 0;
+#pragma unroll
+    for (int i = 0; i < KA; ++i) any |= __shfl(bits, first + i);
+    count = __popcll(any);
+    dense = any ? T + 2 - __ffsll(any) : 0;
 }
 
 template <int MODEL, int KA>
@@ -279,6 +299,8 @@
     double ut[NC];
 #pragma unroll
     for (int i = 0; i < NC; ++i) ut[i] = 0.0;
+    constexpr bool KEYS = wave_emits_keys<MODEL, KA>;
+    unsigned long long near_steps = 0;
 
 #ifdef DPILQR_PHASE_STAMPS
     unsigned long long w_wait = 0, w_t0 = __builtin_amdgcn_s_memtime();
@@ -352,8 +374,14 @@
         }
         const double cr = ref_cost<NS, NC>(x, ut, xf, Q, R, false);
         double cp[PPL > 0 ? PPL : 1];
-#pragma unroll
-        for (int q = 0; q < PPL; ++q) cp[q] = pair_cost_nd<NS>(sxs + (pp[q] & 255) * NS, sxs + ((pp[q] >> 8) & 255) * NS, pp[q] >> 16, radius);
+        bool near_t = false;
+#pragma unroll
+        for (int q = 0; q < PPL; ++q) {
+            bool near_q;
+            cp[q] = pair_cost_nd<NS>(sxs + (pp[q] & 255) * NS, sxs + ((pp[q] >> 8) & 255) * NS, pp[q] >> 16, radius, near_q);
+            near_t = near_t || near_q;
+        }
+        if constexpr (KEYS) wave_key_step(near_steps, near_t);
         DPILQR_LDS_FENCE();
         post_costs(cr, cp, t & 1);
         double xn[NS];
@@ -398,8 +426,14 @@
         for (int c = 0; c < NC; ++c) uz[c] = 0.0;
         const double cr = ref_cost<NS, NC>(x, uz, xf, Qf, R, true);
         double cp[PPL > 0 ? PPL : 1];
-#pragma unroll
-        for (int q = 0; q < PPL; ++q) cp[q] = pair_cost_nd<NS>(sxs + (pp[q] & 255) * NS, sxs + ((pp[q] >> 8) & 255) * NS, pp[q] >> 16, radius);
+        bool near_t = false;
+#pragma unroll
+        for (int q = 0; q < PPL; ++q) {
+            bool near_q;
+            cp[q] = pair_cost_nd<NS>(sxs + (pp[q] & 255) * NS, sxs + ((pp[q] >> 8) & 255) * NS, pp[q] >> 16, radius, near_q);
+            near_t = near_t || near_q;
+        }
+        if constexpr (KEYS) wave_key_step(near_steps, near_t);
         DPILQR_LDS_FENCE();
         post_costs(cr, cp, T & 1);
         wave_sync<NW>();
@@ -421,6 +455,13 @@
     wave_sync<NW>();
     const int acc = ctl[0];
     if (acc < 0) return;
+    if constexpr (KEYS) {
+        if (S.key_count) {
+            int count, dense;
+            wave_key_combine<KA>(near_steps, acc * KA, T, count, dense);
+            if (tid == 0 && S.status[b] == DPILQR_STATUS_ACTIVE) { S.key_count[b] = count; S.key_dense[b] = dense; }
+        }
+    }
     const double* Xa = Xc + ((int64_t)slot * NG + acc) * (int64_t)(T + 1) * n;
     const double* Ua = Uc + ((int64_t)slot * NG + acc) * (int64_t)T * m;
     for (int e = tid; e < (T + 1) * n; e += NTH) Xb[e] = Xa[e];
@@ -437,7 +478,8 @@
 template <int MODEL, int KA>
 __global__ __launch_bounds__(256) void k_rollout_wave(dpilqr_batch_desc D, const double* __restrict__ x0,
                                                       const double* __restrict__ U, double* __restrict__ X,
-                                                      double* __restrict__ Jout) {
+                                                      double* __restrict__ Jout, int32_t* __restrict__ key_count,
+                                                      int32_t* __restrict__ key_dense) {
     using W = WaveRolloutLds<MODEL, KA>;
     constexpr int NS = W::NS, NC = ModelDef<MODEL>::NC, n = W::n, m = KA * NC, NPAIRS = W::NP, NP1 = W::NP1, IPW = W::IPW;
     constexpr PairTable<KA> PT{};
@@ -503,6 +545,8 @@
 #pragma unroll
     for (int i = 0; i < NC; ++i) un[i] = (T > 0) ? Ub[i] : 0.0;
     double J = 0.0;
+    constexpr bool KEYS = wave_emits_keys<MODEL, KA>;
+    unsigned long long near_steps = 0;
     for (int t = 0; t < T; ++t) {
         if (active) store_vec(Xw + (int64_t)t * n, x, NS);
 #pragma unroll
@@ -517,8 +561,14 @@
         if (a == 0 && t > 0) stage_cost(J);
         const double cr = ref_cost<NS, NC>(x, u, xf, Q, R, false);
         double cp[PPL > 0 ? PPL : 1];
-#pragma unroll
-        for (int q = 0; q < PPL; ++q) cp[q] = pair_cost_nd<NS>(sxs + pi[q] * NS, sxs + pj[q] * NS, pnd[q], radius);
+        bool near_t = false;
+#pragma unroll
+        for (int q = 0; q < PPL; ++q) {
+            bool near_q;
+            cp[q] = pair_cost_nd<NS>(sxs + pi[q] * NS, sxs + pj[q] * NS, pnd[q], radius, near_q);
+            near_t = near_t || near_q;
+        }
+        if constexpr (KEYS) wave_key_step(near_steps, near_t);
         DPILQR_LDS_FENCE();
         scr[a] = cr;
 #pragma unroll
@@ -542,8 +592,14 @@
         for (int c = 0; c < NC; ++c) uz[c] = 0.0;
         const double cr = ref_cost<NS, NC>(x, uz, xf, Qf, R, true);
         double cp[PPL > 0 ? PPL : 1];
-#pragma unroll
-        for (int q = 0; q < PPL; ++q) cp[q] = pair_cost_nd<NS>(sxs + pi[q] * NS, sxs + pj[q] * NS, pnd[q], radius);
+        bool near_t = false;
+#pragma unroll
+        for (int q = 0; q < PPL; ++q) {
+            bool near_q;
+            cp[q] = pair_cost_nd<NS>(sxs + pi[q] * NS, sxs + pj[q] * NS, pnd[q], radius, near_q);
+            near_t = near_t || near_q;
+        }
+        if constexpr (KEYS) wave_key_step(near_steps, near_t);
         DPILQR_LDS_FENCE();
         scr[a] = cr;
 #pragma unroll
@@ -553,6 +609,13 @@
         if (a == 0) stage_cost(J);
     }
     if (active && a == 0) Jout[b] = J;
-}
-
-}
+    if constexpr (KEYS) {
+        if (key_count) {
+            int count, dense;
+            wave_key_combine<KA>(near_steps, w * KA, T, count, dense);
+            if (active && a == 0) { key_count[b] = count; key_dense[b] = dense; }
+        }
+    }
+}
+
+}
diff --git a/dpilqr_amd/csrc/launch.hpp b/dpilqr_amd/csrc/launch.hpp
--- a/dpilqr_amd/csrc/launch.hpp
+++ b/dpilqr_amd/csrc/launch.hpp
@@ -137,7 +137,11 @@
                          int min_live, int32_t* key, int32_t* key_dense, hipStream_t st);
 int32_t launch_order_list(const int32_t* src, int32_t* dst, const int32_t* count, const int32_t* key, int T, int cus, int waves,
                           int order, int min_live, hipStream_t st);
-
+int32_t launch_admit_order(int32_t* list, int32_t* dst, int32_t* count, int32_t* next_count, int32_t* admitted, int B, int window,
+                           int32_t* mail, int want_prefix, int64_t* t_admit, const int32_t* fault, const int32_t* item_key, int T,
+                           int cus, int waves, int order, int min_live, hipStream_t st);
+
+bool linesearch_team_serves(const dpilqr_batch_desc& D, int grid_items);
 int32_t launch_linesearch_team(const dpilqr_batch_desc& D, double* X, double* U, const double* K, const double* d,
                                const double* alphas, double* Xc, double* Uc, const SolveState& S, const int32_t* items,
                                const int32_t* n_items, int grid_items, hipStream_t st);
@@ -147,6 +151,8 @@
                        const SolveState& S, const int32_t* items, const int32_t* n_items, int grid_items,
                        hipStream_t st);
 int32_t set_stamp_buffer_forward(void* device_buffer);
+bool forward_emits_keys(const dpilqr_batch_desc& D, int mode, int grid_items);
+extern thread_local bool g_forward_keys;
 int32_t launch_model_op(int op, int32_t n, int32_t ns, const int32_t* model, const double* x, const double* u, double dt,
                         double* o1, double* o2, hipStream_t st);
 int32_t launch_cost_eval(const dpilqr_batch_desc& D, int32_t n_pts, const double* x, const double* u, int32_t terminal,
diff --git a/dpilqr_amd/csrc/solve_state.hpp b/dpilqr_amd/csrc/solve_state.hpp
--- a/dpilqr_amd/csrc/solve_state.hpp
+++ b/dpilqr_amd/csrc/solve_state.hpp
@@ -25,6 +25,8 @@
     double tol;
     const int64_t* t_admit;
     int64_t t_kill_ticks;
+    int32_t* key_count;
+    int32_t* key_dense;
 };
 
 __device__ inline bool solve_time_is_up(const SolveState& S, int b) {
diff --git a/dpilqr_amd/csrc/tu_forward.hip b/dpilqr_amd/csrc/tu_forward.hip
--- a/dpilqr_amd/csrc/tu_forward.hip
+++ b/dpilqr_amd/csrc/tu_forward.hip
@@ -15,17 +15,34 @@
 
 static bool no_wave_ro() { static const bool v = route_flag("DPILQR_FORWARD_GENERIC"); return v; }
 
+static bool forward_takes_big_path(const dpilqr_batch_desc& D, int mode, int ngrp) {
+    const int n = D.k * D.n_s, m = D.k * D.n_c;
+    const int threads = forward_threads(D.k, mode == kModeRollout ? 1 : ngrp);
+    const size_t lds_item = (forward_lds_bytes(n, m, D.k, ngrp) + 15) & ~(size_t)15;
+    return uses_big_path(n) || lds_item > (size_t)kMaxLds || (mode != kModeRollout && (m * n + threads - 1) / threads > kMaxStage);
+}
+
+thread_local bool g_forward_keys = false;
+bool forward_emits_keys(const dpilqr_batch_desc& D, int mode, int grid_items) {
+    if (no_wave_ro() || hint_model(D) != kDoubleInt4D || D.n_s != 4 || D.n_c != 2 || D.k > 5 || D.T + 1 > kWaveKeySteps) return false;
+    if (grid_items <= 0 || forward_takes_big_path(D, mode, mode == kModeRollout ? 1 : DPILQR_N_ALPHA)) return false;
+    return mode == kModeRollout || (mode == kModeLineSearch && !linesearch_team_serves(D, grid_items));
+}
+
 int32_t launch_forward(const dpilqr_batch_desc& D, int mode, const double* x0, double* X, double* U, const double* K,
                        const double* d, const double* alphas, int ngrp, double* Xc, double* Uc, double* Jc,
                        const SolveState& S, const int32_t* items, const int32_t* n_items, int grid_items,
                        hipStream_t st) {
+    g_forward_keys = false;
     if (grid_items <= 0) return DPILQR_OK;
     const int n = D.k * D.n_s, m = D.k * D.n_c;
     int threads = forward_threads(D.k, mode == kModeRollout ? 1 : ngrp);
     if (threads > 256) return fail(DPILQR_EUNSUPPORTED, "k*n_alpha=%d exceeds the 256-thread workgroup of the forward pass", D.k * ngrp);
     const size_t lds_item = (forward_lds_bytes(n, m, D.k, ngrp) + 15) & ~(size_t)15;
-    if (uses_big_path(n) || lds_item > (size_t)kMaxLds || (mode != kModeRollout && (m * n + threads - 1) / threads > kMaxStage))
+    if (forward_takes_big_path(D, mode, ngrp))
         return launch_forward_big_f64(D, mode, x0, X, U, K, d, alphas, ngrp, Xc, Uc, Jc, S, items, n_items, grid_items, st);
+    const bool emit = S.key_count && S.key_dense && forward_emits_keys(D, mode, grid_items) &&
+                      (mode == kModeRollout ? !items : (ngrp == DPILQR_N_ALPHA && items && n_items));
     if (!no_wave_ro() && mode == kModeRollout && hint_model(D) >= 0 && !items) {
         const int model = hint_model(D);
 #define DPILQR_TRY_RO(MODEL, KA)                                                                                    \
@@ -33,8 +50,10 @@
         using WR = WaveRolloutLds<MODEL, KA>;                                                                       \
         const int per_wg = 4 * WR::IPW;                                                                             \
         hipLaunchKernelGGL((k_rollout_wave<MODEL, KA>), dim3((grid_items + per_wg - 1) / per_wg), dim3(256),        \
-                           sizeof(double) * WR::total * 4, st, D, x0, U, X, Jc);                                    \
+                           sizeof(double) * WR::total * 4, st, D, x0, U, X, Jc, emit ? S.key_count : nullptr,       \
+                           emit ? S.key_dense : nullptr);                                                           \
         HIP_TRY(hipGetLastError());                                                                                 \
+        g_forward_keys = emit && wave_emits_keys<MODEL, KA>;                                                        \
         return DPILQR_OK;                                                                                           \
     }
 #define DPILQR_RO_10(MODEL) DPILQR_TRY_RO(MODEL, 1) DPILQR_TRY_RO(MODEL, 2) DPILQR_TRY_RO(MODEL, 3)                \
@@ -66,6 +85,8 @@
             const int32_t rc_t = launch_linesearch_team(D, X, U, K, d, alphas, Xc, Uc, S, items, n_items, grid_items, st);
             if (rc_t != DPILQR_EUNSUPPORTED) return rc_t;
         }
+        SolveState Sw = S;
+        if (!emit) { Sw.key_count = nullptr; Sw.key_dense = nullptr; }
 #define DPILQR_TRY_WAVE(MODEL, KA)                                                                                  \
     if (model == MODEL && D.k == KA && model_ns(MODEL) == D.n_s && model_nc(MODEL) == D.n_c) {                      \
         using WF = WaveFwdLds<MODEL, KA>;                                                                           \
@@ -73,8 +94,9 @@
         int32_t rc_w = allow_lds(k_linesearch_wave<MODEL, KA>, lds_w);                                              \
         if (rc_w) return rc_w;                                                                                      \
         hipLaunchKernelGGL((k_linesearch_wave<MODEL, KA>), dim3((grid_items + WF::IPB - 1) / WF::IPB),              \
-                           dim3(64 * WF::NW * WF::IPB), lds_w, st, D, X, U, K, d, alphas, Xc, Uc, S, items, n_items); \
+                           dim3(64 * WF::NW * WF::IPB), lds_w, st, D, X, U, K, d, alphas, Xc, Uc, Sw, items, n_items); \
         HIP_TRY(hipGetLastError());                                                                                 \
+        g_forward_keys = emit && wave_emits_keys<MODEL, KA>;                                                        \
         return DPILQR_OK;                                                                                           \
     }
 #define DPILQR_WAVE_10(MODEL) DPILQR_TRY_WAVE(MODEL, 1) DPILQR_TRY_WAVE(MODEL, 2) DPILQR_TRY_WAVE(MODEL, 3)        \
diff --git a/dpilqr_amd/csrc/tu_lsteam.hip b/dpilqr_amd/csrc/tu_lsteam.hip
--- a/dpilqr_amd/csrc/tu_lsteam.hip
+++ b/dpilqr_amd/csrc/tu_lsteam.hip
@@ -7,12 +7,16 @@
 
 namespace dpilqr {
 
+bool linesearch_team_serves(const dpilqr_batch_desc& D, int grid_items) {
+    static const bool off = route_flag("DPILQR_LS_NO_TEAM");
+    static const int max_items = route_int("DPILQR_LS_TEAM_MAX", 1024);
+    return !(off || grid_items > max_items || grid_items <= 0 || hint_model(D) < 0);
+}
+
 int32_t launch_linesearch_team(const dpilqr_batch_desc& D, double* X, double* U, const double* K, const double* d,
                                const double* alphas, double* Xc, double* Uc, const SolveState& S, const int32_t* items,
                                const int32_t* n_items, int grid_items, hipStream_t st) {
-    static const bool off = route_flag("DPILQR_LS_NO_TEAM");
-    static const int max_items = route_int("DPILQR_LS_TEAM_MAX", 1024);
-    if (off || grid_items > max_items || grid_items <= 0 || hint_model(D) < 0) return DPILQR_EUNSUPPORTED;
+    if (!linesearch_team_serves(D, grid_items)) return DPILQR_EUNSUPPORTED;
     const int model = hint_model(D);
 #define DPILQR_TRY_LSTEAM(MODEL, KA)                                                                                \
     if (model == MODEL && D.k == KA && model_ns(MODEL) == D.n_s && model_nc(MODEL) == D.n_c) {                      \
diff --git a/dpilqr_amd/csrc/tu_order.hip b/dpilqr_amd/csrc/tu_order.hip
--- a/dpilqr_amd/csrc/tu_order.hip
+++ b/dpilqr_amd/csrc/tu_order.hip
@@ -33,4 +33,13 @@
     return DPILQR_OK;
 }
 
+int32_t launch_admit_order(int32_t* list, int32_t* dst, int32_t* count, int32_t* next_count, int32_t* admitted, int B, int window,
+                           int32_t* mail, int want_prefix, int64_t* t_admit, const int32_t* fault, const int32_t* item_key, int T,
+                           int cus, int waves, int order, int min_live, hipStream_t st) {
+    hipLaunchKernelGGL(k_admit_order, dim3(1), dim3(1024), 0, st, list, dst, count, next_count, admitted, B, window, mail, want_prefix,
+                       t_admit, fault, item_key, T, cus, waves, order, min_live);
+    HIP_TRY(hipGetLastError());
+    return DPILQR_OK;
 }
+
+}
diff --git a/include/dpilqr_hip.h b/include/dpilqr_hip.h
--- a/include/dpilqr_hip.h
+++ b/include/dpilqr_hip.h
@@ -167,6 +167,7 @@
 #include "dpilqr_swarm_advance.h"
 #include "dpilqr_swarm_study.h"
 #include "dpilqr_order.h"
+#include "dpilqr_loop_keys.h"
 #include "dpilqr_nearest.h"
 #include "dpilqr_separated_setup.h"
 
diff --git a/include/dpilqr_loop_keys.h b/include/dpilqr_loop_keys.h
--- /dev/null
+++ b/include/dpilqr_loop_keys.h
@@ -0,0 +1,17 @@
+#ifndef DPILQR_LOOP_KEYS_H
+#define DPILQR_LOOP_KEYS_H
+#ifndef DPILQR_HIP_H
+#error "include dpilqr_hip.h, which includes this header after the types it needs"
+#endif
+
+
+int64_t dpilqr_solve_item_keys_offset(const dpilqr_batch_desc* desc, int32_t window, int32_t gains_in_workspace);
+
+int32_t dpilqr_admit(int32_t* list, int32_t* count, int32_t* next_count, int32_t* admitted, int32_t B, int32_t window, int32_t* mail,
+                     int32_t want_prefix, int64_t* t_admit, const int32_t* fault, void* stream);
+
+int32_t dpilqr_admit_order(int32_t* list, int32_t* count, int32_t* next_count, int32_t* admitted, int32_t B, int32_t window, int32_t* mail,
+                           int32_t want_prefix, int64_t* t_admit, const int32_t* fault, const int32_t* item_keys, int32_t T,
+                           int32_t n_cus, int32_t waves, int32_t order, int32_t min_live, int32_t* out, void* stream);
+
+#endif
```

Result: slower. 938,500 subproblems/s (-9.0%).
